# leaner-forever/SEGS-SLAM

Measured on AMD Instinct MI355X. Metric: mapper train-iters/sec (fwd+bwd raster), higher is better.
Workload: dtype f32; 1 GPU; 1080p_3m: 3000000 Gaussians, 1920x1080, 1 keyframe per GPU, fwd+bwd raster; P=3000000, P_visible=2096178, num_rendered=10472370, instances_binned=7913347, instances_live=6766534, width=1920, height=1080, parallelism=keyframe-dp1, forward=resident (no host sync), hipgraph=off

## Files before the change

include/segs_raster.h:

```cpp
#ifndef SEGS_RASTER_H_
#define SEGS_RASTER_H_

#include <stddef.h>
#include <stdint.h>

#ifdef __cplusplus
extern "C" {
#endif

#define SEGS_OK 0
#define SEGS_ERR_INVALID_ARGUMENT (-1)
#define SEGS_ERR_UNSUPPORTED (-2)
#define SEGS_ERR_ALLOC (-3)

typedef char* (*segs_alloc_fn)(void* ctx, size_t bytes);

const char* segs_last_error(void);

#define SEGS_RASTER_SKIP_NONPOSITIVE_OPACITY 1u
#define SEGS_RASTER_KEEP_DEAD_INSTANCES 2u
#define SEGS_RASTER_GATHER_TILES_TOUCHED 4u
#define SEGS_RASTER_TEST_NARROW_PACK 8u
#define SEGS_RASTER_UNFUSED_BINNING 16u
#define SEGS_RASTER_TIGHT_BINNING 32u
#define SEGS_RASTER_MFMA_MOMENTS 64u
#define SEGS_RASTER_NO_WRITTEN_BYTES 128u
#define SEGS_RASTER_UNPACKED_BACKWARD 256u
uint32_t segs_raster_set_flags(uint32_t flags);

uint32_t* segs_raster_set_status_mirror(uint32_t* host_mapped_status);

size_t segs_geometry_bytes(int P);
size_t segs_image_bytes(int width, int height);
size_t segs_binning_bytes(int num_rendered);

int segs_rasterize_forward(segs_alloc_fn geometry_alloc, void* geometry_ctx,
                           segs_alloc_fn binning_alloc, void* binning_ctx,
                           segs_alloc_fn image_alloc, void* image_ctx,
                           int P, int D, int M,
                           const float* background, int width, int height,
                           const float* means3D, const float* shs, const float* colors_precomp,
                           const float* opacities, const float* scales, float scale_modifier,
                           const float* rotations, const float* cov3D_precomp,
                           const float* viewmatrix, const float* projmatrix, const float* cam_pos,
                           float tan_fovx, float tan_fovy, int prefiltered,
                           float* out_color, int* radii, void* stream, int* num_rendered);

int segs_rasterize_backward(int P, int D, int M, int R,
                            const float* background, int width, int height,
                            const float* means3D, const float* shs, const float* colors_precomp,
                            const float* scales, float scale_modifier, const float* rotations,
                            const float* cov3D_precomp, const float* viewmatrix, const float* projmatrix,
                            const float* campos, float tan_fovx, float tan_fovy, const int* radii,
                            char* geom_buffer, char* binning_buffer, char* image_buffer,
                            const float* dL_dpix, float* dL_dmean2D, float* dL_dconic, float* dL_dopacity,
                            float* dL_dcolor, float* dL_dmean3D, float* dL_dcov3D, float* dL_dsh,
                            float* dL_dscale, float* dL_drot, void* stream);

int segs_visible_filter(int P, int M, int width, int height, const float* means3D, const float* scales,
                        float scale_modifier, const float* rotations, const float* cov3D_precomp,
                        const float* viewmatrix, const float* projmatrix, float tan_fovx, float tan_fovy,
                        int prefiltered, int* radii, void* stream);

int segs_visible_filter_log_scales(int P, int width, int height, const float* means3D, const float* scaling_log, int stride,
                                   const float* rotations, const float* viewmatrix, const float* projmatrix, float tan_fovx,
                                   float tan_fovy, int* radii, void* stream);

int segs_mark_visible(int P, const float* means3D, const float* viewmatrix, const float* projmatrix,
                      uint8_t* present, void* stream);

int segs_project2_image(int P, int D, int M, int width, int height, const float* means3D, const float* shs,
                        const float* colors_precomp, const float* opacities, const float* scales,
                        float scale_modifier, const float* rotations, const float* cov3D_precomp,
                        const float* viewmatrix, const float* projmatrix, const float* cam_pos,
                        float tan_fovx, float tan_fovy, int prefiltered, float* out_color, float* points_image,
                        int* radii, void* stream);

int segs_debug_unpack_geometry(const char* geom_buffer, int P, const int* radii, float* means2D ,
                               float* conic_opacity , float* depths , uint32_t* tiles_touched ,
                               uint32_t* point_offsets , float* rgb , void* stream);
int segs_debug_unpack_binning(const char* binning_buffer, const char* geom_buffer, int P, int R, int width, int height,
                              uint64_t* keys_sorted , uint32_t* point_list , void* stream);
int segs_debug_instance_values(const char* binning_buffer, int R, uint32_t* values , void* stream);
int segs_debug_unpack_image(const char* image_buffer, int width, int height, uint32_t* ranges ,
                            float* final_T , uint32_t* n_contrib , void* stream);

#define SEGS_GEOMETRY_REGIONS 10
int segs_debug_geometry_layout(int P, size_t* offset_and_bytes , int regions);

int segs_debug_preprocess_backward(int P, int width, int height, const float* means3D, const int* radii,
                                   const float* scales, float scale_modifier, const float* rotations,
                                   const float* cov3D_precomp, const float* viewmatrix, const float* projmatrix,
                                   float tan_fovx, float tan_fovy, const float* dL_dmean2D, const float* dL_dconic,
                                   float* dL_dmean3D, float* dL_dcov3D, float* dL_dscale, float* dL_drot, void* stream);

int segs_sort_pairs(const uint64_t* keys_in, const uint32_t* vals_in, uint64_t* keys_out, uint32_t* vals_out,
                    int n, int end_bit, char* temp, void* stream);

size_t segs_resident_binning_bytes(int P, int capacity);
int segs_rasterize_forward_resident(char* geom_buffer, char* binning_buffer, char* image_buffer, int capacity,
                                    int geom_rows, int P, int D, int M, const float* background, int width, int height,
                                    const float* means3D, const float* shs, const float* colors_precomp,
                                    const float* opacities, const float* scales, float scale_modifier,
                                    const float* rotations, const float* cov3D_precomp, const float* viewmatrix,
                                    const float* projmatrix, const float* cam_pos, float tan_fovx, float tan_fovy,
                                    float* out_color, int* radii, uint32_t* status, void* stream);
int segs_rasterize_backward_resident(char* geom_buffer, char* binning_buffer, char* image_buffer, int capacity,
                                     int geom_rows, int P, int D, int M, const float* background, int width, int height,
                                     const float* means3D, const float* shs, const float* scales, float scale_modifier,
                                     const float* rotations, const float* cov3D_precomp, const float* viewmatrix,
                                     const float* projmatrix, const float* campos, float tan_fovx, float tan_fovy,
                                     const int* radii, const float* dL_dpix, float* dL_dmean2D, float* dL_dconic,
                                     float* dL_dopacity, float* dL_dcolor, float* dL_dmean3D, float* dL_dcov3D,
                                     float* dL_dsh, float* dL_dscale, float* dL_drot, void* stream);

typedef struct segs_projection_targets {
  float* records;
  int* radii;
  uint32_t* tiles_touched;
  uint32_t* depth_keys;
  uint32_t* tile_ranges;
  uint32_t* depth_overflow;
  int num_tiles;
  uint32_t flags;
} segs_projection_targets;
int segs_resident_projection_targets(char* geom_buffer, char* binning_buffer, char* image_buffer, int capacity, int geom_rows,
                                     int P, int width, int height, int* radii, uint32_t* status, segs_projection_targets* out);
int segs_rasterize_forward_resident_projected(char* geom_buffer, char* binning_buffer, char* image_buffer, int capacity,
                                              int geom_rows, int P, const float* background, int width, int height,
                                              float* out_color, uint32_t* status, void* stream);

typedef struct segs_depth_outputs {
  float* depth;
  float* alpha;
} segs_depth_outputs;
typedef struct segs_depth_grads {
  const float* dL_ddepth;
  const float* dL_dalpha;
} segs_depth_grads;
int segs_rasterize_forward_depth(segs_alloc_fn geometry_alloc, void* geometry_ctx,
                                 segs_alloc_fn binning_alloc, void* binning_ctx,
                                 segs_alloc_fn image_alloc, void* image_ctx,
                                 int P, int D, int M,
                                 const float* background, int width, int height,
                                 const float* means3D, const float* shs, const float* colors_precomp,
                                 const float* opacities, const float* scales, float scale_modifier,
                                 const float* rotations, const float* cov3D_precomp,
                                 const float* viewmatrix, const float* projmatrix, const float* cam_pos,
                                 float tan_fovx, float tan_fovy, int prefiltered,
                                 float* out_color, int* radii, const segs_depth_outputs* depth_out, void* stream,
                                 int* num_rendered);
int segs_rasterize_backward_depth(int P, int D, int M, int R,
                                  const float* background, int width, int height,
                                  const float* means3D, const float* shs, const float* colors_precomp,
                                  const float* scales, float scale_modifier, const float* rotations,
                                  const float* cov3D_precomp, const float* viewmatrix, const float* projmatrix,
                                  const float* campos, float tan_fovx, float tan_fovy, const int* radii,
                                  char* geom_buffer, char* binning_buffer, char* image_buffer,
                                  const float* dL_dpix, float* dL_dmean2D, float* dL_dconic, float* dL_dopacity,
                                  float* dL_dcolor, float* dL_dmean3D, float* dL_dcov3D, float* dL_dsh,
                                  float* dL_dscale, float* dL_drot, const segs_depth_grads* depth_grads, void* stream);
int segs_rasterize_forward_resident_depth(char* geom_buffer, char* binning_buffer, char* image_buffer, int capacity,
                                          int geom_rows, int P, int D, int M, const float* background, int width, int height,
                                          const float* means3D, const float* shs, const float* colors_precomp,
                                          const float* opacities, const float* scales, float scale_modifier,
                                          const float* rotations, const float* cov3D_precomp, const float* viewmatrix,
                                          const float* projmatrix, const float* cam_pos, float tan_fovx, float tan_fovy,
                                          float* out_color, int* radii, uint32_t* status, const segs_depth_outputs* depth_out,
                                          void* stream);
int segs_rasterize_forward_resident_projected_depth(char* geom_buffer, char* binning_buffer, char* image_buffer, int capacity,
                                                    int geom_rows, int P, const float* background, int width, int height,
                                                    float* out_color, uint32_t* status, const segs_depth_outputs* depth_out,
                                                    void* stream);
int segs_rasterize_backward_resident_depth(char* geom_buffer, char* binning_buffer, char* image_buffer, int capacity,
                                           int geom_rows, int P, int D, int M, const float* background, int width, int height,
                                           const float* means3D, const float* shs, const float* scales, float scale_modifier,
                                           const float* rotations, const float* cov3D_precomp, const float* viewmatrix,
                                           const float* projmatrix, const float* campos, float tan_fovx, float tan_fovy,
                                           const int* radii, const float* dL_dpix, float* dL_dmean2D, float* dL_dconic,
                                           float* dL_dopacity, float* dL_dcolor, float* dL_dmean3D, float* dL_dcov3D,
                                           float* dL_dsh, float* dL_dscale, float* dL_drot, const segs_depth_grads* depth_grads,
                                           void* stream);

typedef struct segs_camera_grads {
  float* dL_dviewmatrix;
  float* dL_dprojmatrix;
  char* temp;
} segs_camera_grads;
size_t segs_camera_grad_temp_bytes(int rows);
int segs_rasterize_backward_camera(int P, int D, int M, int R,
                                   const float* background, int width, int height,
                                   const float* means3D, const float* shs, const float* colors_precomp,
                                   const float* scales, float scale_modifier, const float* rotations,
                                   const float* cov3D_precomp, const float* viewmatrix, const float* projmatrix,
                                   const float* campos, float tan_fovx, float tan_fovy, const int* radii,
                                   char* geom_buffer, char* binning_buffer, char* image_buffer,
                                   const float* dL_dpix, float* dL_dmean2D, float* dL_dconic, float* dL_dopacity,
                                   float* dL_dcolor, float* dL_dmean3D, float* dL_dcov3D, float* dL_dsh,
                                   float* dL_dscale, float* dL_drot, const segs_depth_grads* depth_grads,
                                   const segs_camera_grads* camera_grads, void* stream);
int segs_rasterize_backward_resident_camera(char* geom_buffer, char* binning_buffer, char* image_buffer, int capacity,
                                            int geom_rows, int P, int D, int M, const float* background, int width, int height,
                                            const float* means3D, const float* shs, const float* scales, float scale_modifier,
                                            const float* rotations, const float* cov3D_precomp, const float* viewmatrix,
                                            const float* projmatrix, const float* campos, float tan_fovx, float tan_fovy,
                                            const int* radii, const float* dL_dpix, float* dL_dmean2D, float* dL_dconic,
                                            float* dL_dopacity, float* dL_dcolor, float* dL_dmean3D, float* dL_dcov3D,
                                            float* dL_dsh, float* dL_dscale, float* dL_drot, const segs_depth_grads* depth_grads,
                                            const segs_camera_grads* camera_grads, void* stream);
int segs_debug_preprocess_backward_camera(int P, int width, int height, const float* means3D, const int* radii,
                                          const float* scales, float scale_modifier, const float* rotations,
                                          const float* cov3D_precomp, const float* viewmatrix, const float* projmatrix,
                                          float tan_fovx, float tan_fovy, const float* dL_dmean2D, const float* dL_dconic,
                                          float* dL_dmean3D, float* dL_dcov3D, float* dL_dscale, float* dL_drot,
                                          const float* dL_dz, const segs_camera_grads* camera_grads, void* stream);

int segs_profile_begin(unsigned kernel_mask);
int segs_profile_end(void);
int segs_profile_kernel_count(void);
const char* segs_profile_kernel_name(int id);
int segs_profile_query(int id, double* total_ms, long* launches);

#ifdef __cplusplus
}
#endif
#endif
```

segs-slam_amd/_capi.py:

```python
from __future__ import annotations

import ctypes as C
import os
import subprocess

_HERE = os.path.dirname(os.path.abspath(__file__))
CSRC = os.path.join(_HERE, "csrc")
LIB_PATH = os.environ.get("SEGS_RASTER_LIB") or os.path.join(CSRC, "libsegs_raster.so")

ALLOC_FN = C.CFUNCTYPE(C.c_void_p, C.c_void_p, C.c_size_t)


class NeuralDims(C.Structure):
    _fields_ = [("feat_dim", C.c_int), ("n_offsets", C.c_int), ("appearance_dim", C.c_int), ("use_feat_bank", C.c_int),
                ("add_opacity_dist", C.c_int), ("add_cov_dist", C.c_int), ("add_color_dist", C.c_int)]


class ProjectionTargets(C.Structure):
    _fields_ = [("records", C.c_void_p), ("radii", C.c_void_p), ("tiles_touched", C.c_void_p), ("depth_keys", C.c_void_p),
                ("tile_ranges", C.c_void_p), ("depth_overflow", C.c_void_p), ("num_tiles", C.c_int), ("flags", C.c_uint32)]


class DepthOutputs(C.Structure):
    _fields_ = [("depth", C.c_void_p), ("alpha", C.c_void_p)]


class DepthGrads(C.Structure):
    _fields_ = [("dL_ddepth", C.c_void_p), ("dL_dalpha", C.c_void_p)]


class CameraGrads(C.Structure):
    _fields_ = [("dL_dviewmatrix", C.c_void_p), ("dL_dprojmatrix", C.c_void_p), ("temp", C.c_void_p)]


class DepthLossParamsC(C.Structure):
    _fields_ = [("lambda_depth", C.c_float), ("lambda_alpha", C.c_float), ("alpha_min", C.c_float), ("normalize", C.c_int)]


class DepthSeedParamsC(C.Structure):
    _fields_ = [("stride", C.c_int), ("alpha_max", C.c_float), ("use_front", C.c_int), ("front_abs", C.c_float),
                ("front_rel", C.c_float), ("voxel_size", C.c_float)]


class StereoParamsC(C.Structure):
    _fields_ = [("num_disparities", C.c_int), ("min_disparity", C.c_int), ("P1", C.c_int), ("P2", C.c_int),
                ("uniqueness_ratio", C.c_int), ("paths", C.c_int), ("lr_max_diff", C.c_int), ("median", C.c_int)]


class IntakeCameraC(C.Structure):
    _fields_ = [("in_w", C.c_int), ("in_h", C.c_int), ("out_w", C.c_int), ("out_h", C.c_int),
                ("fx", C.c_float), ("fy", C.c_float), ("cx", C.c_float), ("cy", C.c_float),
                ("k1", C.c_float), ("k2", C.c_float), ("p1", C.c_float), ("p2", C.c_float), ("k3", C.c_float),
                ("rinv", C.c_float * 9), ("nfx", C.c_float), ("nfy", C.c_float), ("ncx", C.c_float), ("ncy", C.c_float)]


class AdamSegment(C.Structure):
    _fields_ = [("offset", C.c_int64), ("count", C.c_int64), ("lr", C.c_double)]

_vp, _i, _f, _sz = C.c_void_p, C.c_int, C.c_float, C.c_size_t
SYMBOLS = {
    "segs_last_error": (C.c_char_p, []),
    "segs_raster_set_flags": (C.c_uint, [C.c_uint]),
    "segs_raster_set_status_mirror": (_vp, [_vp]),
    "segs_training_statis": (_i, [_i, _i] + [_vp] * 9),
    "segs_training_statis_guarded": (_i, [_i, _i] + [_vp] * 10),
    "segs_anchor_growing_temp_bytes": (_sz, [_i, _i]),
    "segs_anchor_growing_level": (_i, [_i, _i, _i, _i] + [_vp] * 7 + [_f, _f, _f, _i] + [_vp] * 5),
    "segs_depth_seed_temp_bytes": (_sz, [_i, _i, _i, _i]),
    "segs_depth_seed": (_i, [_i, _vp, _i, _i, _vp, _vp, _vp, _f, _f, _vp, _vp, _i, _vp, _vp, _vp, _vp, _vp]),
    "segs_neural_set_flags": (C.c_uint, [C.c_uint]),
    "segs_neural_param_layout": (_i, [_vp, _vp, _vp, _vp, _vp]),
    "segs_neural_temp_bytes": (_sz, [_vp, _i]),
    "segs_neural_forward": (_i, [_vp, _i] + [_vp] * 16),
    "segs_neural_forward_projected": (_i, [_vp, _i] + [_vp] * 16 + [_i, _i, _f, _f, _f, _vp, _vp]),
    "segs_neural_backward": (_i, [_vp, _i] + [_vp] * 17 + [_f, _vp, _vp, _vp]),
    "segs_neural_backward_camera": (_i, [_vp, _i] + [_vp] * 17 + [_f, _vp, _vp, _vp, _vp]),
    "segs_geometry_bytes": (_sz, [_i]),
    "segs_debug_geometry_layout": (_i, [_i, _vp, _i]),
    "segs_image_bytes": (_sz, [_i, _i]),
    "segs_binning_bytes": (_sz, [_i]),
    "segs_rasterize_forward": (_i, [ALLOC_FN, _vp, ALLOC_FN, _vp, ALLOC_FN, _vp, _i, _i, _i, _vp, _i, _i, _vp, _vp, _vp,
                                     _vp, _vp, _f, _vp, _vp, _vp, _vp, _vp, _f, _f, _i, _vp, _vp, _vp, C.POINTER(_i)]),
    "segs_rasterize_backward": (_i, [_i, _i, _i, _i, _vp, _i, _i, _vp, _vp, _vp, _vp, _f, _vp, _vp, _vp, _vp, _vp, _f, _f,
                                      _vp, _vp, _vp, _vp, _vp, _vp, _vp, _vp, _vp, _vp, _vp, _vp, _vp, _vp, _vp]),
    "segs_resident_binning_bytes": (_sz, [_i, _i]),
    "segs_rasterize_forward_resident": (_i, [_vp, _vp, _vp, _i, _i, _i, _i, _i, _vp, _i, _i, _vp, _vp, _vp, _vp, _vp, _f, _vp, _vp, _vp,
                                              _vp, _vp, _f, _f, _vp, _vp, _vp, _vp]),
    "segs_resident_projection_targets": (_i, [_vp, _vp, _vp, _i, _i, _i, _i, _i, _vp, _vp, _vp]),
    "segs_rasterize_forward_resident_projected": (_i, [_vp, _vp, _vp, _i, _i, _i, _vp, _i, _i, _vp, _vp, _vp]),
    "segs_rasterize_backward_resident": (_i, [_vp, _vp, _vp, _i, _i, _i, _i, _i, _vp, _i, _i, _vp, _vp, _vp, _f, _vp, _vp, _vp, _vp, _vp,
                                               _f, _f, _vp, _vp, _vp, _vp, _vp, _vp, _vp, _vp, _vp, _vp, _vp, _vp]),
}
for _name in ("segs_rasterize_forward", "segs_rasterize_backward", "segs_rasterize_forward_resident",
              "segs_rasterize_forward_resident_projected", "segs_rasterize_backward_resident"):
    _res, _args = SYMBOLS[_name]
    _at = len(_args) - (2 if _name == "segs_rasterize_forward" else 1)
    SYMBOLS[_name + "_depth"] = (_res, _args[:_at] + [_vp] + _args[_at:])
for _name in ("segs_rasterize_backward", "segs_rasterize_backward_resident"):
    _res, _args = SYMBOLS[_name + "_depth"]
    SYMBOLS[_name + "_camera"] = (_res, _args[:-1] + [_vp] + _args[-1:])
SYMBOLS["segs_camera_grad_temp_bytes"] = (_sz, [_i])
SYMBOLS.update({
    "segs_visible_filter": (_i, [_i, _i, _i, _i, _vp, _vp, _f, _vp, _vp, _vp, _vp, _f, _f, _i, _vp, _vp]),
    "segs_visible_filter_log_scales": (_i, [_i, _i, _i, _vp, _vp, _i, _vp, _vp, _vp, _f, _f, _vp, _vp]),
    "segs_mark_visible": (_i, [_i, _vp, _vp, _vp, _vp, _vp]),
    "segs_project2_image": (_i, [_i, _i, _i, _i, _i, _vp, _vp, _vp, _vp, _vp, _f, _vp, _vp, _vp, _vp, _vp, _f, _f, _i,
                                  _vp, _vp, _vp, _vp]),
    "segs_debug_unpack_geometry": (_i, [_vp, _i, _vp, _vp, _vp, _vp, _vp, _vp, _vp, _vp]),
    "segs_debug_instance_values": (_i, [_vp, _i, _vp, _vp]),
    "segs_debug_unpack_binning": (_i, [_vp, _vp, _i, _i, _i, _i, _vp, _vp, _vp]),
    "segs_debug_unpack_image": (_i, [_vp, _i, _i, _vp, _vp, _vp, _vp]),
    "segs_debug_preprocess_backward": (_i, [_i, _i, _i, _vp, _vp, _vp, _f, _vp, _vp, _vp, _vp, _f, _f, _vp, _vp, _vp,
                                             _vp, _vp, _vp, _vp]),
    "segs_debug_preprocess_backward_camera": (_i, [_i, _i, _i, _vp, _vp, _vp, _f, _vp, _vp, _vp, _vp, _f, _f, _vp, _vp, _vp,
                                                    _vp, _vp, _vp, _vp, _vp, _vp]),
    "segs_sort_pairs": (_i, [_vp, _vp, _vp, _vp, _i, _i, _vp, _vp]),
    "segs_knn_temp_bytes": (_sz, [_i]),
    "segs_knn_mean_dist2": (_i, [_i, _vp, _vp, _vp, _vp]),
    "segs_transform_points": (_i, [_i, _vp, _vp, _vp, _vp]),
    "segs_scale_and_transform_points": (_i, [_i, _f, _vp, _vp, _vp, _vp, _vp, _vp, _vp]),
    "segs_reproject_depths_pinhole": (_i, [_i, _i, _f, _f, _f, _f, _vp, _vp, _vp, _vp]),
    "segs_search_neighborhood_depth": (_i, [_i, _i, _f, _f, _f, _f, _f, _vp, _vp, _vp, _vp, _vp, _vp, _vp]),
    "segs_stereo_sgm_temp_bytes": (_sz, [_i, _i, _i, _i]),
    "segs_stereo_sgm": (_i, [_vp, _i, _i, _vp, _vp, _vp, _vp, _f, _vp, _vp]),
    "segs_rgb_to_gray_u8": (_i, [_i, _i, _vp, _vp, _vp]),
    "segs_debug_stereo_sgm_stages": (_i, [_vp, _i, _i, _vp, _vp, _vp, _vp, _f, _vp] + [_vp] * 6 + [_vp]),
    "segs_undistort_u8": (_i, [_vp, _i, _vp, _vp, _vp, _vp]),
    "segs_undistort_depth": (_i, [_vp, _i, _vp, _f, _i, _vp, _vp]),
    "segs_undistort_mask": (_i, [_vp, _vp, _vp]),
    "segs_debug_undistort_map": (_i, [_vp, _vp, _vp]),
    "segs_resize_levels": (_i, [_i, _i, _i, _vp, _i, _vp, _vp, _vp, _vp]),
    "segs_l1_ssim_temp_bytes": (_sz, [_i, _i]),
    "segs_l1_ssim_tile_rows": (_i, [_i, _i]),
    "segs_l1_ssim_loss": (_i, [_vp, _vp, _i, _i, _f, _vp, _vp, _vp, _vp]),
    "segs_freq_pyramid": (_i, [_vp, _i, _i, _i, _i, _vp, _vp, _vp, _vp]),
    "segs_spectrum_magnitude": (_i, [_vp, _sz, _vp, _vp]),
    "segs_freq_temp_bytes": (_sz, [_i, _i, _vp, _vp]),
    "segs_freq_spectrum_loss": (_i, [_i, _i, _vp, _vp, _vp, _vp, _vp, _vp, _vp, _vp, _vp]),
    "segs_freq_pyramid_backward_add": (_i, [_vp, _i, _i, _i, _i, _vp, _vp, _vp, _vp]),
    "segs_freq_plan_create": (_i, [_i, _i, _i, _vp, _f, _vp]),
    "segs_freq_plan_destroy": (None, [_vp]),
    "segs_freq_plan_levels": (_i, [_vp, _vp, _vp, _vp]),
    "segs_freq_target_floats": (_sz, [_vp]),
    "segs_freq_target": (_i, [_vp, _vp, _vp, _vp]),
    "segs_freq_loss": (_i, [_vp, _vp, _vp, _vp, _vp, _vp, _vp]),
    "segs_depth_target_floats": (_sz, [_i, _i]),
    "segs_depth_target": (_i, [_vp, _i, _i, _f, _f, _vp, _vp]),
    "segs_depth_loss_temp_bytes": (_sz, [_i, _i]),
    "segs_depth_loss": (_i, [_vp, _vp, _vp, _i, _i, _vp, _vp, _vp, _vp, _vp, _vp, _vp]),
    "segs_adam_step": (_i, [_vp, _vp, _vp, _vp, _vp, _i, C.c_double, C.c_double, C.c_double, C.c_int64, _f, _i, _vp]),
    "segs_adam_step_guarded": (_i, [_vp, _vp, _vp, _vp, _vp, _i, C.c_double, C.c_double, C.c_double, C.c_int64, _f, _i, _vp, _vp]),
    "segs_adam_step_device": (_i, [_vp, _vp, _vp, _vp, _vp, _i, C.c_double, C.c_double, C.c_double, _vp, _i, _f, _i, _vp, _vp]),
    "segs_adam_step_graph": (_i, [_vp, _vp, _vp, _vp, _vp, _i, _vp, C.c_double, C.c_double, C.c_double, _vp, _f, _i, _vp, _vp]),
    "segs_set_doubles": (_i, [_vp, _vp, _i, _vp]),
    "segs_profile_begin": (_i, [C.c_uint]),
    "segs_profile_end": (_i, []),
    "segs_profile_kernel_count": (_i, []),
    "segs_profile_kernel_name": (C.c_char_p, [_i]),
    "segs_profile_query": (_i, [_i, C.POINTER(C.c_double), C.POINTER(C.c_long)]),
})

_lib = None


def build(force: bool = False) -> str:
    cmd = ["make", "-C", CSRC, "-s", "-j4"] + (["-B"] if force else [])
    subprocess.check_call(cmd)
    return LIB_PATH


def lib() -> C.CDLL:
    global _lib
    if _lib is None:
        if not os.path.exists(LIB_PATH):
            raise RuntimeError(
                f"{LIB_PATH} is missing: the HIP extension must be built (python -c 'import __graft_entry__ as g; "
                "g.build()' or make -C segs-slam_amd/csrc). There is no CPU fallback.")
        import torch
        l = C.CDLL(LIB_PATH)
        for name, (res, args) in SYMBOLS.items():
            try:
                fn = getattr(l, name)
            except AttributeError as e:
                raise RuntimeError(f"libsegs_raster.so does not export {name}") from e
            fn.restype = res
            fn.argtypes = args
        _lib = l
    return _lib


class raster_flags:

    def __init__(self, flags: int, status_mirror=None, clear_mirror: bool = True):
        self.flags, self.status_mirror, self.clear_mirror = flags, status_mirror, clear_mirror

    def __enter__(self):
        self.old = lib().segs_raster_set_flags(self.flags)
        if self.status_mirror is not None:
            _lib.segs_raster_set_status_mirror(self.status_mirror)

    def __exit__(self, *exc):
        _lib.segs_raster_set_flags(self.old)
        if self.clear_mirror:
            _lib.segs_raster_set_status_mirror(None)


class SegsError(RuntimeError):
    pass


def check(status: int, what: str) -> None:
    if status != 0:
        msg = lib().segs_last_error()
        raise SegsError(f"{what} failed with status {status}: {msg.decode() if msg else ''}")
```

segs-slam_amd/csrc/capi.hip:

```cpp
#include <hip/hip_runtime.h>
#include <cstdio>
#include <cstdlib>
#include <algorithm>
#include <cstring>
#include <string>
#include <vector>
#include "../../include/segs_raster.h"
#include "gs_layout.h"
#include "kernels.h"
#include "capi_args.h"

using namespace segs;

namespace {
thread_local std::string g_err;
}
int segs::set_error(int code, const char* what) {
  g_err = what;
  return code;
}
int segs::set_hip_error(hipError_t e, const char* where) {
  g_err = std::string(where) + ": " + hipGetErrorString(e);
  return (int)e > 0 ? (int)e : 1;
}

namespace {

thread_local uint32_t g_flags = 0u;
thread_local uint32_t* g_status_mirror = nullptr;

int fail(int code, const char* what) { return segs::set_error(code, what); }
int hip_fail(hipError_t e, const char* where) { return segs::set_hip_error(e, where); }
#define HIP_TRY(expr)                                   \
  do {                                                  \
    hipError_t _e = (expr);                             \
    if (_e != hipSuccess) return hip_fail(_e, #expr);   \
  } while (0)
#define LAUNCH_TRY(name)                                \
  do {                                                  \
    hipError_t _e = hipGetLastError();                  \
    if (_e != hipSuccess) return hip_fail(_e, name);    \
  } while (0)

enum KernelId { K_PREPROCESS_FWD = 0, K_SCAN, K_DUPLICATE, K_RADIX_COUNT, K_RADIX_SCAN, K_RADIX_SCATTER, K_RANGES,
                K_RENDER_FWD, K_RENDER_BWD, K_PREPROCESS_BWD, K_MEMSET, K_COUNT };
const char* const kKernelNames[K_COUNT] = {"preprocess_fwd_kernel", "scan_block_sums_kernel", "duplicate_with_keys_kernel",
                                           "radix_count_kernel", "radix_scan_kernel", "radix_scatter_kernel",
                                           "identify_tile_ranges_kernel", "render_fwd_kernel", "render_bwd_kernel",
                                           "preprocess_bwd_kernel", "memset"};
struct Profiler {
  unsigned mask = 0;
  std::vector<hipEvent_t> pool;
  size_t used = 0;
  struct Span { int id; size_t e0, e1; };
  std::vector<Span> spans;
  double total_ms[K_COUNT] = {0};
  long count[K_COUNT] = {0};
  hipEvent_t get() {
    if (used == pool.size()) { hipEvent_t e; if (hipEventCreate(&e) != hipSuccess) return nullptr; pool.push_back(e); }
    return pool[used++];
  }
} g_prof;
struct ProfScope {
  int id; hipStream_t st; size_t e0 = 0; bool on;
  ProfScope(int id_, hipStream_t st_) : id(id_), st(st_), on((g_prof.mask >> id_) & 1u) {
    if (on) { e0 = g_prof.used; hipEvent_t e = g_prof.get(); if (e) (void)hipEventRecord(e, st); else on = false; }
  }
  ~ProfScope() {
    if (on) { size_t e1 = g_prof.used; hipEvent_t e = g_prof.get(); if (e) { (void)hipEventRecord(e, st); g_prof.spans.push_back({id, e0, e1}); } }
  }
};
#define PROF(id) ProfScope _prof_scope_##id(id, st)

uint32_t getHigherMsb(uint32_t n) {
  uint32_t msb = sizeof(n) * 4, step = msb;
  while (step > 1) {
    step /= 2;
    if (n >> msb) msb += step; else msb -= step;
  }
  if (n >> msb) msb++;
  return msb;
}

int count_chunk_tiles(int nblocks) {
#ifdef SEGS_MEASURE
  static const int chunk_override = [] { const char* e = getenv("SEGS_COUNT_CHUNK"); const int v = e ? atoi(e) : 0; return (v == 1 || v == 2 || v == 4) ? v : 0; }();
  if (chunk_override > 0) return chunk_override;
#endif
  return nblocks <= 256 ? 1 : (nblocks <= 2048 ? 2 : SORT_COUNT_CHUNK_TILES);
}

int check_tile_grid(const View& V) {
  if (V.gx > 0xFFFFu || V.gy > 0xFFFFu) return fail(SEGS_ERR_INVALID_ARGUMENT, "image too large for 16-bit tile coordinates");
  return SEGS_OK;
}
int check_colour_and_shape(const Gaussians& g, const View& V) {
  if (!g.colors_precomp && (!g.shs || !V.cam_pos || g.M <= 0 || g.D < 0 || (g.D + 1) * (g.D + 1) > g.M || g.D > 3))
    return fail(SEGS_ERR_INVALID_ARGUMENT, "need colors_precomp, or shs + cam_pos with (D+1)^2 <= M, D <= 3");
  if (!g.cov3D_precomp && (!g.scales || !g.rotations)) return fail(SEGS_ERR_INVALID_ARGUMENT, "need scales+rotations or cov3D_precomp");
  return SEGS_OK;
}

template <typename K, int BITS>
int sort_pairs_digits(char* bin, const BinningLayout& L, int n, const SortOptions& o, hipStream_t st) {
  if (n <= 0) return SEGS_OK;
  uint32_t* n_live = (uint32_t*)(bin + L.n_live);
  const int end_bit = o.end_bit, passes = (end_bit + BITS - 1) / BITS;
  int side = sort_first_side(end_bit, BITS);
  uint32_t* tile_prefix = (uint32_t*)(bin + L.tile_prefix);
  uint32_t* chunk_hist = (uint32_t*)(bin + L.chunk_hist);
  uint32_t* digit_totals = (uint32_t*)(bin + L.digit_totals);
  const int chunk_tiles = count_chunk_tiles(L.nblocks);
  const int nchunks = (L.nblocks + chunk_tiles - 1) / chunk_tiles;
  for (int p = 0; p < passes; p++) {
    const K* kin = (p == 0 && o.first_keys) ? (const K*)o.first_keys : (const K*)(bin + L.keys[side]);
    const uint32_t* vin = (const uint32_t*)(bin + L.vals[side]);
    K* kout = (K*)(bin + L.keys[side ^ 1]);
    uint32_t* vout = (uint32_t*)(bin + L.vals[side ^ 1]);
    const int shift = BITS * p;
    const int drop = o.drop_dead && p == 0;
    const uint32_t* n_in = (o.drop_dead && p > 0) ? n_live : o.n_dev;
    const int nbits = std::min(BITS, end_bit - shift);
    { PROF(K_RADIX_COUNT);
    radix_count_kernel<K, BITS><<<(nchunks + 7) / 8 * 8, SORT_THREADS, 0, st>>>(kin, n, shift, o.dmin, o.dbits, tile_prefix, chunk_hist, L.nblocks, nchunks, n_in, drop, chunk_tiles, nbits);
    }
    LAUNCH_TRY("radix_count_kernel");
    const bool last = p == passes - 1;
    { PROF(K_RADIX_SCAN);
    radix_scan_kernel<<<1 << BITS, 256, 0, st>>>(chunk_hist, nchunks, digit_totals);
    }
    LAUNCH_TRY("radix_scan_kernel");
    if (o.iota_vals && p == 0) vin = nullptr;
    const int scatter_grid = (L.nblocks + 7) / 8 * 8;
    uint2* fr = last ? o.ranges : nullptr;
    uint32_t* fs = last ? o.status : nullptr;
    uint32_t* fm = last ? o.status_mirror : nullptr;
    const int wk = (last && !o.keep_sorted_keys) ? 0 : 1;
    { PROF(K_RADIX_SCATTER);
    bool gathered = false;
    if constexpr (sizeof(K) == 4 && BITS <= 9) {
      if (o.aux_in && o.aux_final && last) {
        radix_scatter_kernel<K, BITS, true><<<scatter_grid, SORT_THREADS, 0, st>>>(kin, vin, kout, vout, n, shift, o.dmin, o.dbits, tile_prefix, chunk_hist,
                                                                        digit_totals, L.nblocks, nchunks, n_in, drop,
                                                                        drop ? n_live : nullptr, o.aux_in, o.aux_final, nbits, chunk_tiles, 0, fr, fs, fm, wk);
        gathered = true;
      }
    }
    if (!gathered)
      radix_scatter_kernel<K, BITS, false><<<scatter_grid, SORT_THREADS, 0, st>>>(kin, vin, kout, vout, n, shift, o.dmin, o.dbits, tile_prefix, chunk_hist,
                                                                       digit_totals, L.nblocks, nchunks, n_in, drop,
                                                                       drop ? n_live : nullptr, (o.pack_shift > 0 && p == 0) ? o.aux_in : nullptr, nullptr,
                                                                       nbits, chunk_tiles, (p == 0) ? o.pack_shift : 0, fr, fs, fm, wk);
    }
    LAUNCH_TRY("radix_scatter_kernel");
    side ^= 1;
  }
  return SEGS_OK;
}
template <typename K>
int sort_pairs(char* bin, const BinningLayout& L, int n, const SortOptions& o, hipStream_t st) {
  if constexpr (sizeof(K) == 4) {
    if (o.digit_bits == 9) return sort_pairs_digits<K, 9>(bin, L, n, o, st);
    if (o.digit_bits == 11) return sort_pairs_digits<K, 11>(bin, L, n, o, st);
  }
  return sort_pairs_digits<K, 8>(bin, L, n, o, st);
}

bool drop_dead_instances() { return (g_flags & SEGS_RASTER_KEEP_DEAD_INSTANCES) == 0u; }
uint32_t resident_k1_flags() { return drop_dead_instances() ? PREPROCESS_TIGHT_RECT : 0u; }

int run_preprocess(const Geom& G, const Gaussians& g, const View& V, int* radii, const K1Targets& k1, hipStream_t st) {
  { PROF(K_PREPROCESS_FWD);
  preprocess_fwd_kernel<<<G.L.nblocks, 256, 0, st>>>(g.P, g.means3D, g.kernel_scales(), g.scale_modifier, g.rotations, g.opacities, g.colors_precomp,
                                                     g.cov3D_precomp, V.viewmatrix, V.projmatrix, V.width, V.height, V.tan_fovx, V.tan_fovy,
                                                     V.focal_x, V.focal_y, V.gx, V.gy, radii, G.rec(), G.bin(), G.block_sums(),
                                                     G.block_sums() + (G.L.nblocks + 1), g.shs, g.D, g.M, V.cam_pos, G.clamped(),
                                                     g_flags | k1.extra_flags, k1.depth_keys, k1.depth_vals, k1.ranges, (int)V.tiles,
                                                     k1.depth_overflow, G.touched());
  }
  LAUNCH_TRY("preprocess_fwd_kernel");
  return SEGS_OK;
}

int run_binning(const Scratch& S, const View& V, const BinningMode& mode, hipStream_t st) {
  const Geom& G = S.G; const BinningLayout& BL = S.BL; const GaussSortLayout& GS = S.GS;
  char* const bin = S.bin; uint2* const ranges = S.ranges();
  const int P = G.L.P, n_cap = BL.R;
  const uint32_t* const n_dev = S.status;
  uint32_t* const total_out = S.status ? S.status : (uint32_t*)(bin + GS.block_sums) + G.L.nblocks;
  const int bit = (int)getHigherMsb(V.tiles);
  char* gbin = bin + GS.base;
  const BinningLayout& GL = GS.inner;
  if (!mode.k1_keys) { PROF(K_DUPLICATE);
  const DepthSortInput in = depth_sort_input(bin, GS, mode.dbits, mode.digit_bits);
  make_depth_keys_kernel<<<G.L.nblocks, 256, 0, st>>>(P, G.bin(), mode.dcull, in.keys, in.vals, ranges, (int)V.tiles);
  }
  LAUNCH_TRY("make_depth_keys_kernel");
  const bool drop_culled = mode.k1_keys != nullptr;
  int idx_bits = 1;
  while (idx_bits < 32 && ((uint64_t)1 << idx_bits) < (uint64_t)P) idx_bits++;
  int pack_shift = (32 - idx_bits >= 6 && !(g_flags & SEGS_RASTER_GATHER_TILES_TOUCHED)) ? idx_bits : 0;
  if (pack_shift && (g_flags & SEGS_RASTER_TEST_NARROW_PACK)) pack_shift = 30;
  SortOptions depth_sort;
  depth_sort.end_bit = mode.dbits; depth_sort.digit_bits = mode.digit_bits;
  depth_sort.dmin = mode.dmin; depth_sort.dbits = mode.dbits;
  depth_sort.drop_dead = drop_culled; depth_sort.iota_vals = true;
  depth_sort.aux_in = G.touched(); depth_sort.aux_final = pack_shift ? nullptr : G.offsets(); depth_sort.pack_shift = pack_shift;
  depth_sort.first_keys = mode.k1_keys;
  int rc = sort_pairs<uint32_t>(gbin, GL, P, depth_sort, st);
  if (rc) return rc;
  uint32_t* order = (uint32_t*)(gbin + GL.vals[0]);
  const uint32_t* ng_dev = drop_culled ? (const uint32_t*)(gbin + GL.n_live) : nullptr;
  uint32_t* sums2 = (uint32_t*)(bin + GS.block_sums);
  uint32_t* first_owner = (uint32_t*)(bin + GS.first_owner);
  const int prefix_wgs = (P + 256 * PREFIX_ROWS_PER_WG - 1) / (256 * PREFIX_ROWS_PER_WG);
  { PROF(K_SCAN);
  ordered_block_sums_kernel<<<prefix_wgs, 256, 0, st>>>(P, pack_shift ? G.touched() : G.offsets(), nullptr, sums2, G.offsets(), ng_dev, order, pack_shift);
  }
  LAUNCH_TRY("ordered_block_sums_kernel");
#ifdef SEGS_MEASURE
  static const bool no_wide = getenv("SEGS_NO_WIDE_DIGIT") != nullptr;
#else
  constexpr bool no_wide = false;
#endif
  SortOptions tile_sort;
  tile_sort.end_bit = bit;
  tile_sort.digit_bits = (!no_wide && bit <= 11 && BL.nblocks <= SORT_WIDE_MAX_TILES) ? 11 : 8;
  tile_sort.n_dev = n_dev; tile_sort.drop_dead = mode.drop_dead;
  const int tpasses = (bit + tile_sort.digit_bits - 1) / tile_sort.digit_bits;
  const int side = sort_first_side(bit, tile_sort.digit_bits);
  { PROF(K_SCAN);
  ordered_offsets_kernel<<<prefix_wgs, 256, 0, st>>>(P, sums2, G.offsets(), total_out, ng_dev, first_owner,
                                                      (uint32_t)(n_cap / EMIT_SLOTS_PER_WG + 2));
  }
  LAUNCH_TRY("ordered_offsets_kernel");
  const bool unfused = (g_flags & SEGS_RASTER_UNFUSED_BINNING) != 0u;
  { PROF(K_DUPLICATE);
  duplicate_with_keys_kernel<<<(n_cap + EMIT_SLOTS_PER_WG - 1) / EMIT_SLOTS_PER_WG, 256, 0, st>>>(P, n_cap, G.rec(), order, G.offsets(),
                                                                    (uint32_t*)(bin + BL.keys[side]), (uint32_t*)(bin + BL.vals[side]), V.gx, n_dev,
                                                                    mode.drop_dead ? 1 : 0, ng_dev, first_owner);
  }
  LAUNCH_TRY("duplicate_with_keys_kernel");
  const bool fused_ranges = !unfused && tpasses >= 2;
  if (fused_ranges) {
    tile_sort.ranges = ranges;
    tile_sort.status = n_dev ? total_out : nullptr;
    tile_sort.status_mirror = n_dev ? g_status_mirror : nullptr;
    tile_sort.keep_sorted_keys = n_dev == nullptr;
  }
  rc = sort_pairs<uint32_t>(bin, BL, n_cap, tile_sort, st);
  if (rc) return rc;
  if (!fused_ranges) { PROF(K_RANGES);
  identify_tile_ranges_kernel<<<(n_cap + 256 * RANGE_KEYS_PER_THREAD - 1) / (256 * RANGE_KEYS_PER_THREAD), 256, 0, st>>>(n_cap, (const uint32_t*)(bin + BL.keys[0]), ranges, n_dev,
                                                                   n_dev ? total_out : nullptr, n_dev ? g_status_mirror : nullptr,
                                                                   mode.drop_dead ? (const uint32_t*)(bin + BL.n_live) : nullptr);
  }
  LAUNCH_TRY("identify_tile_ranges_kernel");
  return SEGS_OK;
}

int launch_render_fwd(const Scratch& S, const View& V, const float* background, float* out_color, const segs_depth_outputs* dout,
                      hipStream_t st) {
  PROF(K_RENDER_FWD);
  if (dout && (dout->depth || dout->alpha))
    render_fwd_depth_kernel<<<V.tiles, 256, 0, st>>>(S.ranges(), S.point_list(), V.width, V.height, S.G.rec(), background, S.final_T(),
                                                     S.n_contrib(), out_color, dout->depth, dout->alpha);
  else
    render_fwd_kernel<<<V.tiles, 256, 0, st>>>(S.ranges(), S.point_list(), V.width, V.height, S.G.rec(), background, S.final_T(), S.n_contrib(),
                                               out_color);
  LAUNCH_TRY("render_fwd_kernel");
  return SEGS_OK;
}

int launch_render_bwd(const Scratch& S, const View& V, const float* background, const float* dL_dpix, const segs_depth_grads* dgrad,
                      uint8_t* written, hipStream_t st) {
  PROF(K_RENDER_BWD);
  const uint32_t grid = (V.tiles + 7) / 8 * 32;
  if (dgrad && (dgrad->dL_ddepth || dgrad->dL_dalpha)) {
    render_bwd_depth_kernel<<<grid, 64, 0, st>>>(S.ranges(), S.point_list(), V.width, V.height, S.G.rec(), background, S.final_T(),
                                                 S.n_contrib(), dL_dpix, S.G.gacc(), V.tiles, dgrad->dL_ddepth, dgrad->dL_dalpha, written);
    LAUNCH_TRY("render_bwd_depth_kernel");
    return SEGS_OK;
  }
  static const bool mfma_env = [] { const char* e = getenv("SEGS_RENDER_BWD_MFMA"); return e && e[0] == '1'; }();
  ((mfma_env || (g_flags & SEGS_RASTER_MFMA_MOMENTS)) ? render_bwd_mfma_kernel : render_bwd_kernel)<<<grid, 64, 0, st>>>(
      S.ranges(), S.point_list(), V.width, V.height, S.G.rec(), background, S.final_T(), S.n_contrib(), dL_dpix, S.G.gacc(), V.tiles, written);
  LAUNCH_TRY("render_bwd_kernel");
  return SEGS_OK;
}

int camera_grads_begin(const segs_camera_grads* cam, const float* shs, bool empty, hipStream_t st, bool* live) {
  *live = false;
  if (!cam) return SEGS_OK;
  if (!cam->dL_dviewmatrix || !cam->dL_dprojmatrix || !cam->temp) return fail(SEGS_ERR_INVALID_ARGUMENT, "segs_camera_grads: null field");
  if (shs) return fail(SEGS_ERR_INVALID_ARGUMENT, "camera gradients need colors_precomp: the SH colours depend on campos, which they do not cover");
  if (empty) {
    HIP_TRY(hipMemsetAsync(cam->dL_dviewmatrix, 0, 16 * sizeof(float), st));
    HIP_TRY(hipMemsetAsync(cam->dL_dprojmatrix, 0, 16 * sizeof(float), st));
    return SEGS_OK;
  }
  *live = true;
  return SEGS_OK;
}
float* camera_partials(const segs_camera_grads* cam) { return (float*)align_ptr(cam->temp); }
int camera_grads_finish(const segs_camera_grads* cam, int nblocks, hipStream_t st) {
  camera_grad_reduce_kernel<<<1, 960, 0, st>>>(camera_partials(cam), nblocks, cam->dL_dviewmatrix, cam->dL_dprojmatrix);
  LAUNCH_TRY("camera_grad_reduce_kernel");
  return SEGS_OK;
}

int launch_preprocess_bwd(const Gaussians& g, const View& V, const int* radii, const GradOutputs& o, const PerGaussianBwd& m, hipStream_t st) {
  const bool depth = m.depth || m.dz_in;
  auto* const kernel = m.cam ? (depth ? preprocess_bwd_kernel<true, true> : preprocess_bwd_kernel<false, true>)
                             : (depth ? preprocess_bwd_kernel<true, false> : preprocess_bwd_kernel<false, false>);
  const int nblocks = (g.P + 255) / 256;
  if (m.packed) {
    auto* const packed = m.cam ? (depth ? preprocess_bwd_packed_kernel<true, true> : preprocess_bwd_packed_kernel<false, true>)
                               : (depth ? preprocess_bwd_packed_kernel<true, false> : preprocess_bwd_packed_kernel<false, false>);
    packed<<<nblocks, 256, 0, st>>>(g.P, g.means3D, radii, g.kernel_scales(), g.rotations, g.scale_modifier, g.cov3D_precomp, V.viewmatrix,
                                    V.projmatrix, V.focal_x, V.focal_y, V.tan_fovx, V.tan_fovy, m.gacc, (float)V.width, (float)V.height,
                                    o.dL_dmean2D, o.dL_dconic, o.dL_dopacity, o.dL_dcolor, o.dL_dmean3D, o.dL_dcov3D, o.dL_dscale, o.dL_drot,
                                    m.cam ? camera_partials(m.cam) : nullptr, m.written);
    LAUNCH_TRY("preprocess_bwd_packed_kernel");
    return m.cam ? camera_grads_finish(m.cam, nblocks, st) : SEGS_OK;
  }
  kernel<<<nblocks, 256, 0, st>>>(g.P, g.means3D, radii, g.kernel_scales(), g.rotations, g.scale_modifier, g.cov3D_precomp, V.viewmatrix,
                                  V.projmatrix, V.focal_x, V.focal_y, V.tan_fovx, V.tan_fovy, m.gacc, (float)V.width, (float)V.height,
                                  o.dL_dmean2D, o.dL_dconic, o.dL_dopacity, o.dL_dcolor, o.dL_dmean3D, o.dL_dcov3D, o.dL_dscale, o.dL_drot,
                                  m.clean_gacc ? 1 : 0, m.dz_in, m.cam ? camera_partials(m.cam) : nullptr, m.written);
  LAUNCH_TRY("preprocess_bwd_kernel");
  return m.cam ? camera_grads_finish(m.cam, nblocks, st) : SEGS_OK;
}

int rasterize_forward(const Allocators& A, const Gaussians& g, const View& V, const float* background, float* out_color, int* radii,
                      const segs_depth_outputs* dout, hipStream_t st, int* num_rendered) {
  const int P = g.P;
  if (!A.geometry_alloc || !A.binning_alloc || !A.image_alloc) return fail(SEGS_ERR_INVALID_ARGUMENT, "null allocator callback");
  if (P < 0 || V.width <= 0 || V.height <= 0) return fail(SEGS_ERR_INVALID_ARGUMENT, "bad P / image size");
  if (P > MAX_GAUSSIANS) return fail(SEGS_ERR_INVALID_ARGUMENT, "P exceeds 2^28 Gaussians (sort values carry a 4-bit quadrant mask)");
  if (!background || !out_color || !V.viewmatrix || !V.projmatrix || !num_rendered) return fail(SEGS_ERR_INVALID_ARGUMENT, "null required pointer");
  if (P > 0 && (!g.means3D || !g.opacities)) return fail(SEGS_ERR_INVALID_ARGUMENT, "null means3D/opacities");
  if (P > 0)
    if (int rc = check_colour_and_shape(g, V)) return rc;
  if (int rc = check_tile_grid(V)) return rc;

  Scratch S{};
  char* geom_raw = A.geometry_alloc(A.geometry_ctx, geom_layout(P).total);
  S.IL = image_layout(V.width, V.height);
  char* img_raw = A.image_alloc(A.image_ctx, S.IL.total);
  if (!geom_raw || !img_raw) return fail(SEGS_ERR_ALLOC, "allocator callback returned null");
  S.G = geom_at(geom_raw, P);
  S.img = align_ptr(img_raw);
  const Geom& G = S.G;
  if (!radii) radii = G.radii_internal();

  int R = 0;
  uint32_t hdr[3] = {0u, 0u, 0u};
  const bool tight = (g_flags & SEGS_RASTER_TIGHT_BINNING) != 0u;
  bool fast_keys = tight;
  if (P > 0) {
    K1Targets k1;
    k1.extra_flags = tight ? PREPROCESS_TIGHT_RECT : 0u;
    if (fast_keys) { k1.depth_keys = (uint32_t*)G.bin(); k1.ranges = S.ranges(); }
    int rc = run_preprocess(G, g, V, radii, k1, st);
    if (rc) return rc;
    { PROF(K_SCAN);
    scan_block_sums_kernel<<<1, 1024, 0, st>>>(G.block_sums(), G.L.nblocks, G.block_sums() + (G.L.nblocks + 1), G.num_rendered());
    }
    LAUNCH_TRY("scan_block_sums_kernel");
    HIP_TRY(hipMemcpyAsync(hdr, G.num_rendered(), sizeof(hdr), hipMemcpyDeviceToHost, st));
    HIP_TRY(hipStreamSynchronize(st));
    R = (int)hdr[0];
    if (R < 0) return fail(SEGS_ERR_INVALID_ARGUMENT, "num_rendered overflows int32");
    if (fast_keys && R > 0 && (hdr[2] - DEPTH_KEY_MIN) >= ((1u << DEPTH_KEY_BITS) - 1u)) {
      fast_keys = false;
      K1Targets exact;
      exact.extra_flags = PREPROCESS_TIGHT_RECT;
      rc = run_preprocess(G, g, V, radii, exact, st);
      if (rc) return rc;
    }
  }
  S.BL = binning_layout(R);
  S.GS = gauss_sort_layout(R, P);
  char* bin_raw = A.binning_alloc(A.binning_ctx, S.GS.total);
  if (!bin_raw) return fail(SEGS_ERR_ALLOC, "binning allocator returned null");
  S.bin = align_ptr(bin_raw);

  if (R == 0) {
    PROF(K_MEMSET);
    HIP_TRY(hipMemsetAsync(S.ranges(), 0, (size_t)V.gx * V.gy * sizeof(uint2), st));
  }
  if (R > 0) {
    const BinningMode mode = fast_keys ? BinningMode::resident_keys((const uint32_t*)G.bin(), tight)
                                       : BinningMode::exact_range(hdr[1], hdr[2], tight);
    if (int rc = run_binning(S, V, mode, st)) return rc;
  }
  if (int rc = launch_render_fwd(S, V, background, out_color, dout, st)) return rc;
  *num_rendered = R;
  return SEGS_OK;
}

int open_resident(const ScratchBuffers& B, int P, const View& V, uint32_t* status, bool others_present, const Gaussians* k1, Scratch* S) {
  if (P <= 0 || B.capacity <= 0 || V.width <= 0 || V.height <= 0) return fail(SEGS_ERR_INVALID_ARGUMENT, "bad sizes");
  if (B.geom_rows < P) return fail(SEGS_ERR_INVALID_ARGUMENT, "geom_rows (rows the geometry buffer was sized for) must be >= P");
  if (B.geom_rows > MAX_GAUSSIANS) return fail(SEGS_ERR_INVALID_ARGUMENT, "P exceeds 2^28 Gaussians");
  if (!B.geom_buffer || !B.binning_buffer || !B.image_buffer || !status || !others_present) return fail(SEGS_ERR_INVALID_ARGUMENT, "null required pointer");
  if (k1)
    if (int rc = check_colour_and_shape(*k1, V)) return rc;
  if (int rc = check_tile_grid(V)) return rc;
  *S = carve(B, P, V, status);
  return SEGS_OK;
}

int rasterize_forward_resident(const ScratchBuffers& B, int P, const Gaussians* k1, const View& V, const float* background, float* out_color,
                               int* radii, uint32_t* status, const segs_depth_outputs* dout, hipStream_t st) {
  Scratch S{};
  const bool others_present = background && out_color && (!k1 || (V.viewmatrix && V.projmatrix && k1->means3D && k1->opacities));
  if (int rc = open_resident(B, P, V, status, others_present, k1, &S)) return rc;
  const DepthSortInput keys = resident_depth_sort_input(S.bin, S.GS);
  if (k1) {
    K1Targets t;
    t.depth_keys = keys.keys; t.depth_vals = keys.vals; t.ranges = S.ranges();
    t.extra_flags = resident_k1_flags(); t.depth_overflow = status + 2;
    if (int rc = run_preprocess(S.G, *k1, V, radii ? radii : S.G.radii_internal(), t, st)) return rc;
  }
  if (int rc = run_binning(S, V, BinningMode::resident_keys(keys.keys, drop_dead_instances()), st)) return rc;
  return launch_render_fwd(S, V, background, out_color, dout, st);
}

int rasterize_backward(const Gaussians& g, const View& V, const ScratchBuffers& B, const BackwardInputs& in, const GradOutputs& o,
                       GaccCleaning cleaning, hipStream_t st) {
  const int P = g.P, R = B.capacity;
  const bool self_clean = cleaning == SELF_CLEAN;
  if (P < 0 || R < 0 || V.width <= 0 || V.height <= 0) return fail(SEGS_ERR_INVALID_ARGUMENT, "bad sizes");
  if (B.geom_rows < P) return fail(SEGS_ERR_INVALID_ARGUMENT, "geom_rows must be >= P");
  bool cam_live = false;
  if (int rc = camera_grads_begin(in.cam, g.shs, P == 0 || R == 0, st, &cam_live)) return rc;
  if (P == 0) return SEGS_OK;
  if (g.shs && (!V.cam_pos || !o.dL_dsh || g.M <= 0)) return fail(SEGS_ERR_INVALID_ARGUMENT, "SH path needs campos, dL_dsh and M > 0");
  if (!B.geom_buffer || !B.binning_buffer || !B.image_buffer || !in.dL_dpix || !in.background || !g.means3D || !V.viewmatrix || !V.projmatrix)
    return fail(SEGS_ERR_INVALID_ARGUMENT, "null required pointer");
  if (!o.dL_dmean2D || !o.dL_dopacity || !o.dL_dcolor || !o.dL_dmean3D || (g.cov3D_precomp && !o.dL_dcov3D))
    return fail(SEGS_ERR_INVALID_ARGUMENT, "null gradient output");
  if (!g.cov3D_precomp && (!g.scales || !g.rotations || !o.dL_dscale || !o.dL_drot))
    return fail(SEGS_ERR_INVALID_ARGUMENT, "need scales+rotations (+ their gradient outputs) or cov3D_precomp");
  uint32_t* const no_status = nullptr;
  const Scratch S = carve(B, P, V, no_status);
  const Geom& G = S.G;
  const int* radii = in.radii ? in.radii : G.radii_internal();

  if (!self_clean) { PROF(K_MEMSET);
  HIP_TRY(hipMemsetAsync(G.gacc(), 0, (size_t)P * GACC_DWORDS * 4, st));
  }
  PerGaussianBwd m;
  m.gacc = G.gacc(); m.depth = in.dgrad && in.dgrad->dL_ddepth; m.clean_gacc = self_clean;
  if (cam_live) m.cam = in.cam;
  m.written = (self_clean && !(g_flags & SEGS_RASTER_NO_WRITTEN_BYTES)) ? G.written() : nullptr;
  m.packed = m.written && !(g_flags & SEGS_RASTER_UNPACKED_BACKWARD);
  if (R > 0)
    if (int rc = launch_render_bwd(S, V, in.background, in.dL_dpix, in.dgrad, m.written, st)) return rc;
  { PROF(K_PREPROCESS_BWD);
  if (int rc = launch_preprocess_bwd(g, V, radii, o, m, st)) return rc;
  }
  if (g.shs) {
    sh_backward_kernel<<<G.L.nblocks, 256, 0, st>>>(P, g.means3D, radii, g.shs, g.D, g.M, V.cam_pos, G.clamped(), o.dL_dcolor, o.dL_dmean3D, o.dL_dsh);
    LAUNCH_TRY("sh_backward_kernel");
  }
  return SEGS_OK;
}

int visible_filter(const Gaussians& g, const View& V, int log_scale_stride, int* radii, hipStream_t st) {
  if (g.P < 0 || V.width <= 0 || V.height <= 0) return fail(SEGS_ERR_INVALID_ARGUMENT, "bad sizes");
  if (g.P == 0) return SEGS_OK;
  if (!g.means3D || !V.viewmatrix || !V.projmatrix || !radii) return fail(SEGS_ERR_INVALID_ARGUMENT, "null required pointer");
  if (!g.cov3D_precomp && (!g.scales || !g.rotations)) return fail(SEGS_ERR_INVALID_ARGUMENT, "need scales+rotations or cov3D_precomp");
  visible_filter_kernel<<<(g.P + 255) / 256, 256, 0, st>>>(g.P, g.means3D, g.kernel_scales(), g.scale_modifier, g.rotations, g.cov3D_precomp,
                                                           V.viewmatrix, V.projmatrix, V.width, V.height, V.tan_fovx, V.tan_fovy, V.focal_x,
                                                           V.focal_y, V.gx, V.gy, radii, log_scale_stride);
  LAUNCH_TRY("visible_filter_kernel");
  return SEGS_OK;
}

int debug_preprocess_backward(const Gaussians& g, const View& V, const int* radii, const GradOutputs& o, const float* dL_dz,
                              const segs_camera_grads* cam, hipStream_t st) {
  bool cam_live = false;
  if (int rc = camera_grads_begin(cam, g.shs, g.P <= 0, st, &cam_live)) return rc;
  if (g.P <= 0) return SEGS_OK;
  if (!g.means3D || !radii || !V.viewmatrix || !V.projmatrix || !o.dL_dmean2D || !o.dL_dconic || !o.dL_dmean3D || !o.dL_dcov3D)
    return fail(SEGS_ERR_INVALID_ARGUMENT, "null pointer");
  PerGaussianBwd m;
  if (cam_live) { m.dz_in = dL_dz; m.cam = cam; }
  return launch_preprocess_bwd(g, V, radii, o, m, st);
}

}

extern "C" {

const char* segs_last_error(void) { return g_err.c_str(); }

uint32_t* segs_raster_set_status_mirror(uint32_t* host_mapped_status) {
  uint32_t* old = g_status_mirror;
  g_status_mirror = host_mapped_status;
  return old;
}

uint32_t segs_raster_set_flags(uint32_t flags) {
  const uint32_t old = g_flags;
  g_flags = flags;
  return old;
}

size_t segs_geometry_bytes(int P) { return geom_layout(P < 0 ? 0 : P).total; }
size_t segs_image_bytes(int width, int height) { return image_layout(width, height).total; }

int segs_debug_geometry_layout(int P, size_t* offset_and_bytes, int regions) {
  if (P < 0 || !offset_and_bytes || regions != SEGS_GEOMETRY_REGIONS) return fail(SEGS_ERR_INVALID_ARGUMENT, "bad P / region count");
  const GeomLayout g = geom_layout(P);
  const size_t p = (size_t)P;
  const size_t v[SEGS_GEOMETRY_REGIONS][2] = {
      {g.rec, p * REC_DWORDS * 4}, {g.bin, p * sizeof(BinInfo)}, {g.offsets, p * 4}, {g.radii_internal, p * 4},
      {g.block_sums, (size_t)(g.nblocks + 1) * 4 * 3}, {g.clamped, p * 4}, {g.num_rendered, 64}, {g.gacc, p * GACC_DWORDS * 4},
      {g.touched, p * 4}, {g.written, p}};
  for (int i = 0; i < SEGS_GEOMETRY_REGIONS; i++) { offset_and_bytes[2 * i] = v[i][0]; offset_and_bytes[2 * i + 1] = v[i][1]; }
  return SEGS_OK;
}
size_t segs_binning_bytes(int num_rendered) { return binning_layout(num_rendered < 0 ? 0 : num_rendered).total; }

int segs_rasterize_forward(segs_alloc_fn geometry_alloc, void* geometry_ctx, segs_alloc_fn binning_alloc, void* binning_ctx,
                           segs_alloc_fn image_alloc, void* image_ctx, int P, int D, int M, const float* background,
                           int width, int height, const float* means3D, const float* shs, const float* colors_precomp,
                           const float* opacities, const float* scales, float scale_modifier, const float* rotations,
                           const float* cov3D_precomp, const float* viewmatrix, const float* projmatrix,
                           const float* cam_pos, float tan_fovx, float tan_fovy, int prefiltered, float* out_color,
                           int* radii, void* stream, int* num_rendered) {
  (void)prefiltered;
  return rasterize_forward(Allocators{geometry_alloc, geometry_ctx, binning_alloc, binning_ctx, image_alloc, image_ctx},
                           Gaussians{P, means3D, scales, scale_modifier, rotations, cov3D_precomp, D, M, shs, colors_precomp, opacities},
                           camera_view(width, height, viewmatrix, projmatrix, cam_pos, tan_fovx, tan_fovy), background, out_color, radii,
                           NO_DEPTH_OUTPUTS, (hipStream_t)stream, num_rendered);
}

int segs_rasterize_forward_depth(segs_alloc_fn geometry_alloc, void* geometry_ctx, segs_alloc_fn binning_alloc, void* binning_ctx,
                                 segs_alloc_fn image_alloc, void* image_ctx, int P, int D, int M, const float* background,
                                 int width, int height, const float* means3D, const float* shs, const float* colors_precomp,
                                 const float* opacities, const float* scales, float scale_modifier, const float* rotations,
                                 const float* cov3D_precomp, const float* viewmatrix, const float* projmatrix,
                                 const float* cam_pos, float tan_fovx, float tan_fovy, int prefiltered, float* out_color,
                                 int* radii, const segs_depth_outputs* depth_out, void* stream, int* num_rendered) {
  (void)prefiltered;
  return rasterize_forward(Allocators{geometry_alloc, geometry_ctx, binning_alloc, binning_ctx, image_alloc, image_ctx},
                           Gaussians{P, means3D, scales, scale_modifier, rotations, cov3D_precomp, D, M, shs, colors_precomp, opacities},
                           camera_view(width, height, viewmatrix, projmatrix, cam_pos, tan_fovx, tan_fovy), background, out_color, radii,
                           depth_out, (hipStream_t)stream, num_rendered);
}

int segs_rasterize_backward(int P, int D, int M, int R, const float* background, int width, int height,
                            const float* means3D, const float* shs, const float* colors_precomp, const float* scales,
                            float scale_modifier, const float* rotations, const float* cov3D_precomp,
                            const float* viewmatrix, const float* projmatrix, const float* campos, float tan_fovx,
                            float tan_fovy, const int* radii, char* geom_buffer, char* binning_buffer, char* image_buffer,
                            const float* dL_dpix, float* dL_dmean2D, float* dL_dconic, float* dL_dopacity, float* dL_dcolor,
                            float* dL_dmean3D, float* dL_dcov3D, float* dL_dsh, float* dL_dscale, float* dL_drot, void* stream) {
  (void)colors_precomp;
  return rasterize_backward(Gaussians{P, means3D, scales, scale_modifier, rotations, cov3D_precomp, D, M, shs},
                            camera_view(width, height, viewmatrix, projmatrix, campos, tan_fovx, tan_fovy),
                            ScratchBuffers{geom_buffer, binning_buffer, image_buffer, R, P},
                            BackwardInputs{background, radii, dL_dpix, NO_DEPTH_GRADS, NO_CAMERA_GRADS},
                            GradOutputs{dL_dmean2D, dL_dconic, dL_dmean3D, dL_dcov3D, dL_dscale, dL_drot, dL_dopacity, dL_dcolor, dL_dsh},
                            MEMSET_PER_CALL, (hipStream_t)stream);
}

int segs_rasterize_backward_depth(int P, int D, int M, int R, const float* background, int width, int height,
                                  const float* means3D, const float* shs, const float* colors_precomp, const float* scales,
                                  float scale_modifier, const float* rotations, const float* cov3D_precomp,
                                  const float* viewmatrix, const float* projmatrix, const float* campos, float tan_fovx,
                                  float tan_fovy, const int* radii, char* geom_buffer, char* binning_buffer, char* image_buffer,
                                  const float* dL_dpix, float* dL_dmean2D, float* dL_dconic, float* dL_dopacity, float* dL_dcolor,
                                  float* dL_dmean3D, float* dL_dcov3D, float* dL_dsh, float* dL_dscale, float* dL_drot,
                                  const segs_depth_grads* depth_grads, void* stream) {
  (void)colors_precomp;
  return rasterize_backward(Gaussians{P, means3D, scales, scale_modifier, rotations, cov3D_precomp, D, M, shs},
                            camera_view(width, height, viewmatrix, projmatrix, campos, tan_fovx, tan_fovy),
                            ScratchBuffers{geom_buffer, binning_buffer, image_buffer, R, P},
                            BackwardInputs{background, radii, dL_dpix, depth_grads, NO_CAMERA_GRADS},
                            GradOutputs{dL_dmean2D, dL_dconic, dL_dmean3D, dL_dcov3D, dL_dscale, dL_drot, dL_dopacity, dL_dcolor, dL_dsh},
                            MEMSET_PER_CALL, (hipStream_t)stream);
}

size_t segs_camera_grad_temp_bytes(int rows) { return align_up((size_t)((rows < 0 ? 0 : rows) + 255) / 256 * CAM_SUMS * sizeof(float)) + ALIGN; }

int segs_rasterize_backward_camera(int P, int D, int M, int R, const float* background, int width, int height,
                                   const float* means3D, const float* shs, const float* colors_precomp, const float* scales,
                                   float scale_modifier, const float* rotations, const float* cov3D_precomp,
                                   const float* viewmatrix, const float* projmatrix, const float* campos, float tan_fovx,
                                   float tan_fovy, const int* radii, char* geom_buffer, char* binning_buffer, char* image_buffer,
                                   const float* dL_dpix, float* dL_dmean2D, float* dL_dconic, float* dL_dopacity, float* dL_dcolor,
                                   float* dL_dmean3D, float* dL_dcov3D, float* dL_dsh, float* dL_dscale, float* dL_drot,
                                   const segs_depth_grads* depth_grads, const segs_camera_grads* camera_grads, void* stream) {
  (void)colors_precomp;
  return rasterize_backward(Gaussians{P, means3D, scales, scale_modifier, rotations, cov3D_precomp, D, M, shs},
                            camera_view(width, height, viewmatrix, projmatrix, campos, tan_fovx, tan_fovy),
                            ScratchBuffers{geom_buffer, binning_buffer, image_buffer, R, P},
                            BackwardInputs{background, radii, dL_dpix, depth_grads, camera_grads},
                            GradOutputs{dL_dmean2D, dL_dconic, dL_dmean3D, dL_dcov3D, dL_dscale, dL_drot, dL_dopacity, dL_dcolor, dL_dsh},
                            MEMSET_PER_CALL, (hipStream_t)stream);
}

int segs_visible_filter(int P, int M, int width, int height, const float* means3D, const float* scales,
                        float scale_modifier, const float* rotations, const float* cov3D_precomp, const float* viewmatrix,
                        const float* projmatrix, float tan_fovx, float tan_fovy, int prefiltered, int* radii, void* stream) {
  (void)M; (void)prefiltered;
  return visible_filter(Gaussians{P, means3D, scales, scale_modifier, rotations, cov3D_precomp},
                        camera_view(width, height, viewmatrix, projmatrix, NO_CAM_POS, tan_fovx, tan_fovy), 0, radii, (hipStream_t)stream);
}

int segs_visible_filter_log_scales(int P, int width, int height, const float* means3D, const float* scaling_log, int stride,
                                   const float* rotations, const float* viewmatrix, const float* projmatrix, float tan_fovx,
                                   float tan_fovy, int* radii, void* stream) {
  if (stride < 3 || !scaling_log || !rotations) return fail(SEGS_ERR_INVALID_ARGUMENT, "need log-scales (stride >= 3) and rotations");
  return visible_filter(Gaussians{P, means3D, scaling_log, 1.0f, rotations},
                        camera_view(width, height, viewmatrix, projmatrix, NO_CAM_POS, tan_fovx, tan_fovy), stride, radii, (hipStream_t)stream);
}

int segs_mark_visible(int P, const float* means3D, const float* viewmatrix, const float* projmatrix, uint8_t* present, void* stream) {
  (void)projmatrix;
  hipStream_t st = (hipStream_t)stream;
  if (P < 0) return fail(SEGS_ERR_INVALID_ARGUMENT, "bad P");
  if (P == 0) return SEGS_OK;
  if (!means3D || !viewmatrix || !present) return fail(SEGS_ERR_INVALID_ARGUMENT, "null required pointer");
  mark_visible_kernel<<<(P + 255) / 256, 256, 0, st>>>(P, means3D, viewmatrix, present);
  LAUNCH_TRY("mark_visible_kernel");
  return SEGS_OK;
}

int segs_debug_unpack_geometry(const char* geom_buffer, int P, const int* radii, float* means2D, float* conic_opacity,
                               float* depths, uint32_t* tiles_touched, uint32_t* point_offsets, float* rgb, void* stream) {
  hipStream_t st = (hipStream_t)stream;
  if (P <= 0) return SEGS_OK;
  if (!geom_buffer || !means2D || !conic_opacity || !depths || !tiles_touched) return fail(SEGS_ERR_INVALID_ARGUMENT, "null pointer");
  Geom G = geom_at(const_cast<char*>(geom_buffer), P);
  if (!radii) radii = G.radii_internal();
  unpack_geometry_kernel<<<(P + 255) / 256, 256, 0, st>>>(P, G.rec(), G.bin(), radii, means2D, conic_opacity, depths, tiles_touched, rgb);
  LAUNCH_TRY("unpack_geometry_kernel");
  if (point_offsets) {
    point_offsets_kernel<<<1, 1024, 0, st>>>(P, G.bin(), point_offsets);
    LAUNCH_TRY("point_offsets_kernel");
  }
  return SEGS_OK;
}

int segs_debug_unpack_binning(const char* binning_buffer, const char* geom_buffer, int P, int R, int width, int height,
                              uint64_t* keys_sorted, uint32_t* point_list, void* stream) {
  (void)width; (void)height;
  hipStream_t st = (hipStream_t)stream;
  if (R <= 0) return SEGS_OK;
  if (!binning_buffer || (keys_sorted && (!geom_buffer || P <= 0))) return fail(SEGS_ERR_INVALID_ARGUMENT, "null pointer");
  const BinningLayout BL = binning_layout(R);
  const char* bin = align_ptr(binning_buffer);
  if (keys_sorted) {
    const Geom G = geom_at(const_cast<char*>(geom_buffer), P);
    rebuild_keys_kernel<<<(R + 255) / 256, 256, 0, st>>>(R, (const uint32_t*)(bin + BL.keys[0]), (const uint32_t*)(bin + BL.vals[0]),
                                                        G.bin(), keys_sorted);
    LAUNCH_TRY("rebuild_keys_kernel");
  }
  if (point_list) {
    strip_mask_kernel<<<(R + 255) / 256, 256, 0, st>>>(R, (const uint32_t*)(bin + BL.vals[0]), point_list);
    LAUNCH_TRY("strip_mask_kernel");
  }
  return SEGS_OK;
}

int segs_debug_instance_values(const char* binning_buffer, int R, uint32_t* values, void* stream) {
  if (R <= 0) return SEGS_OK;
  if (!binning_buffer || !values) return fail(SEGS_ERR_INVALID_ARGUMENT, "null pointer");
  const BinningLayout BL = binning_layout(R);
  HIP_TRY(hipMemcpyAsync(values, align_ptr(binning_buffer) + BL.vals[0], (size_t)R * 4, hipMemcpyDeviceToDevice, (hipStream_t)stream));
  return SEGS_OK;
}

int segs_debug_unpack_image(const char* image_buffer, int width, int height, uint32_t* ranges, float* final_T,
                            uint32_t* n_contrib, void* stream) {
  hipStream_t st = (hipStream_t)stream;
  if (!image_buffer) return fail(SEGS_ERR_INVALID_ARGUMENT, "null pointer");
  const ImageLayout IL = image_layout(width, height);
  const char* img = align_ptr(image_buffer);
  const size_t tiles = image_view(width, height).tiles;
  if (ranges) {
    HIP_TRY(hipMemcpyAsync(ranges, img + IL.ranges, tiles * 8, hipMemcpyDeviceToDevice, st));
    normalize_ranges_kernel<<<(int)((tiles + 255) / 256), 256, 0, st>>>((int)tiles, (uint2*)ranges);
    LAUNCH_TRY("normalize_ranges_kernel");
  }
  if (final_T) HIP_TRY(hipMemcpyAsync(final_T, img + IL.final_T, (size_t)width * height * 4, hipMemcpyDeviceToDevice, st));
  if (n_contrib) HIP_TRY(hipMemcpyAsync(n_contrib, img + IL.n_contrib, (size_t)width * height * 4, hipMemcpyDeviceToDevice, st));
  return SEGS_OK;
}

int segs_debug_preprocess_backward(int P, int width, int height, const float* means3D, const int* radii, const float* scales,
                                   float scale_modifier, const float* rotations, const float* cov3D_precomp,
                                   const float* viewmatrix, const float* projmatrix, float tan_fovx, float tan_fovy,
                                   const float* dL_dmean2D, const float* dL_dconic, float* dL_dmean3D, float* dL_dcov3D,
                                   float* dL_dscale, float* dL_drot, void* stream) {
  return debug_preprocess_backward(Gaussians{P, means3D, scales, scale_modifier, rotations, cov3D_precomp},
                                   camera_view(width, height, viewmatrix, projmatrix, NO_CAM_POS, tan_fovx, tan_fovy), radii,
                                   GradOutputs{const_cast<float*>(dL_dmean2D), const_cast<float*>(dL_dconic), dL_dmean3D, dL_dcov3D, dL_dscale, dL_drot}, NO_DL_DZ,
                                   NO_CAMERA_GRADS, (hipStream_t)stream);
}

int segs_debug_preprocess_backward_camera(int P, int width, int height, const float* means3D, const int* radii, const float* scales,
                                          float scale_modifier, const float* rotations, const float* cov3D_precomp,
                                          const float* viewmatrix, const float* projmatrix, float tan_fovx, float tan_fovy,
                                          const float* dL_dmean2D, const float* dL_dconic, float* dL_dmean3D, float* dL_dcov3D,
                                          float* dL_dscale, float* dL_drot, const float* dL_dz, const segs_camera_grads* camera_grads,
                                          void* stream) {
  return debug_preprocess_backward(Gaussians{P, means3D, scales, scale_modifier, rotations, cov3D_precomp},
                                   camera_view(width, height, viewmatrix, projmatrix, NO_CAM_POS, tan_fovx, tan_fovy), radii,
                                   GradOutputs{const_cast<float*>(dL_dmean2D), const_cast<float*>(dL_dconic), dL_dmean3D, dL_dcov3D, dL_dscale, dL_drot}, dL_dz, camera_grads,
                                   (hipStream_t)stream);
}

int segs_sort_pairs(const uint64_t* keys_in, const uint32_t* vals_in, uint64_t* keys_out, uint32_t* vals_out, int n,
                    int end_bit, char* temp, void* stream) {
  hipStream_t st = (hipStream_t)stream;
  if (n < 0 || end_bit <= 0 || end_bit > 64) return fail(SEGS_ERR_INVALID_ARGUMENT, "bad n / end_bit");
  if (n == 0) return SEGS_OK;
  if (!keys_in || !vals_in || !keys_out || !vals_out || !temp) return fail(SEGS_ERR_INVALID_ARGUMENT, "null pointer");
  const BinningLayout BL = binning_layout(n);
  char* bin = align_ptr(temp);
  SortOptions sort;
  sort.end_bit = end_bit; sort.dbits = 32;
  const int side = sort_first_side(end_bit, sort.digit_bits);
  HIP_TRY(hipMemcpyAsync(bin + BL.keys[side], keys_in, (size_t)n * 8, hipMemcpyDeviceToDevice, st));
  HIP_TRY(hipMemcpyAsync(bin + BL.vals[side], vals_in, (size_t)n * 4, hipMemcpyDeviceToDevice, st));
  int rc = sort_pairs<uint64_t>(bin, BL, n, sort, st);
  if (rc) return rc;
  HIP_TRY(hipMemcpyAsync(keys_out, bin + BL.keys[0], (size_t)n * 8, hipMemcpyDeviceToDevice, st));
  HIP_TRY(hipMemcpyAsync(vals_out, bin + BL.vals[0], (size_t)n * 4, hipMemcpyDeviceToDevice, st));
  return SEGS_OK;
}

int segs_project2_image(int P, int D, int M, int width, int height, const float* means3D, const float* shs,
                        const float* colors_precomp, const float* opacities, const float* scales, float scale_modifier,
                        const float* rotations, const float* cov3D_precomp, const float* viewmatrix, const float* projmatrix,
                        const float* cam_pos, float tan_fovx, float tan_fovy, int prefiltered, float* out_color,
                        float* points_image, int* radii, void* stream) {
  (void)prefiltered;
  hipStream_t st = (hipStream_t)stream;
  if (P < 0 || width <= 0 || height <= 0) return fail(SEGS_ERR_INVALID_ARGUMENT, "bad sizes");
  if (P == 0) return SEGS_OK;
  if (!colors_precomp && (!shs || !cam_pos || M <= 0)) return fail(SEGS_ERR_INVALID_ARGUMENT, "need colors_precomp or shs + cam_pos");
  if (!means3D || !opacities || !viewmatrix || !projmatrix || !out_color || !points_image || !radii)
    return fail(SEGS_ERR_INVALID_ARGUMENT, "null required pointer");
  const GeomLayout GL = geom_layout(P);
  char* raw = nullptr;
  HIP_TRY(hipMallocAsync((void**)&raw, GL.total + (size_t)P * 4 * 8, st));
  Geom G = geom_at(raw, P);
  float* tmp = (float*)(align_ptr(raw) + GL.total - ALIGN);
  int rc = run_preprocess(G, Gaussians{P, means3D, scales, scale_modifier, rotations, cov3D_precomp, D, M, shs, colors_precomp, opacities},
                          camera_view(width, height, viewmatrix, projmatrix, cam_pos, tan_fovx, tan_fovy), radii, K1Targets(), st);
  if (rc == SEGS_OK) {
    unpack_geometry_kernel<<<(P + 255) / 256, 256, 0, st>>>(P, G.rec(), G.bin(), radii, points_image, tmp, tmp + (size_t)4 * P,
                                                            (uint32_t*)(tmp + (size_t)5 * P), out_color);
    hipError_t e = hipGetLastError();
    if (e != hipSuccess) rc = hip_fail(e, "unpack_geometry_kernel");
  }
  hipError_t fe = hipFreeAsync(raw, st);
  if (rc == SEGS_OK && fe != hipSuccess) return hip_fail(fe, "hipFreeAsync");
  return rc;
}


size_t segs_resident_binning_bytes(int P, int capacity) { return gauss_sort_layout(capacity < 0 ? 0 : capacity, P < 0 ? 0 : P).total; }

int segs_rasterize_forward_resident(char* geom_buffer, char* binning_buffer, char* image_buffer, int capacity, int geom_rows, int P, int D, int M,
                                    const float* background, int width, int height, const float* means3D, const float* shs,
                                    const float* colors_precomp, const float* opacities, const float* scales, float scale_modifier,
                                    const float* rotations, const float* cov3D_precomp, const float* viewmatrix,
                                    const float* projmatrix, const float* cam_pos, float tan_fovx, float tan_fovy, float* out_color,
                                    int* radii, uint32_t* status, void* stream) {
  const Gaussians g{P, means3D, scales, scale_modifier, rotations, cov3D_precomp, D, M, shs, colors_precomp, opacities};
  return rasterize_forward_resident(ScratchBuffers{geom_buffer, binning_buffer, image_buffer, capacity, geom_rows}, P, &g,
                                    camera_view(width, height, viewmatrix, projmatrix, cam_pos, tan_fovx, tan_fovy), background, out_color,
                                    radii, status, NO_DEPTH_OUTPUTS, (hipStream_t)stream);
}

int segs_rasterize_forward_resident_depth(char* geom_buffer, char* binning_buffer, char* image_buffer, int capacity, int geom_rows, int P,
                                          int D, int M, const float* background, int width, int height, const float* means3D,
                                          const float* shs, const float* colors_precomp, const float* opacities, const float* scales,
                                          float scale_modifier, const float* rotations, const float* cov3D_precomp,
                                          const float* viewmatrix, const float* projmatrix, const float* cam_pos, float tan_fovx,
                                          float tan_fovy, float* out_color, int* radii, uint32_t* status,
                                          const segs_depth_outputs* depth_out, void* stream) {
  const Gaussians g{P, means3D, scales, scale_modifier, rotations, cov3D_precomp, D, M, shs, colors_precomp, opacities};
  return rasterize_forward_resident(ScratchBuffers{geom_buffer, binning_buffer, image_buffer, capacity, geom_rows}, P, &g,
                                    camera_view(width, height, viewmatrix, projmatrix, cam_pos, tan_fovx, tan_fovy), background, out_color,
                                    radii, status, depth_out, (hipStream_t)stream);
}

int segs_resident_projection_targets(char* geom_buffer, char* binning_buffer, char* image_buffer, int capacity, int geom_rows, int P,
                                     int width, int height, int* radii, uint32_t* status, segs_projection_targets* out) {
  if (!out) return fail(SEGS_ERR_INVALID_ARGUMENT, "bad sizes");
  const View V = image_view(width, height);
  Scratch S{};
  const bool nothing_else_required = true;
  if (int rc = open_resident(ScratchBuffers{geom_buffer, binning_buffer, image_buffer, capacity, geom_rows}, P, V, status, nothing_else_required,
                             K1_RAN_AT_PRODUCER, &S))
    return rc;
  out->records = S.G.rec();
  out->radii = radii ? radii : S.G.radii_internal();
  out->tiles_touched = S.G.touched();
  out->depth_keys = resident_depth_sort_input(S.bin, S.GS).keys;
  out->tile_ranges = (uint32_t*)S.ranges();
  out->depth_overflow = status + 2;
  out->num_tiles = (int)V.tiles;
  out->flags = resident_k1_flags();
  return SEGS_OK;
}

int segs_rasterize_forward_resident_projected(char* geom_buffer, char* binning_buffer, char* image_buffer, int capacity, int geom_rows, int P,
                                              const float* background, int width, int height, float* out_color, uint32_t* status,
                                              void* stream) {
  return rasterize_forward_resident(ScratchBuffers{geom_buffer, binning_buffer, image_buffer, capacity, geom_rows}, P, K1_RAN_AT_PRODUCER,
                                    image_view(width, height), background, out_color, NO_RADII, status, NO_DEPTH_OUTPUTS, (hipStream_t)stream);
}

int segs_rasterize_forward_resident_projected_depth(char* geom_buffer, char* binning_buffer, char* image_buffer, int capacity,
                                                    int geom_rows, int P, const float* background, int width, int height,
                                                    float* out_color, uint32_t* status, const segs_depth_outputs* depth_out,
                                                    void* stream) {
  return rasterize_forward_resident(ScratchBuffers{geom_buffer, binning_buffer, image_buffer, capacity, geom_rows}, P, K1_RAN_AT_PRODUCER,
                                    image_view(width, height), background, out_color, NO_RADII, status, depth_out, (hipStream_t)stream);
}

int segs_rasterize_backward_resident(char* geom_buffer, char* binning_buffer, char* image_buffer, int capacity, int geom_rows, int P, int D, int M,
                                     const float* background, int width, int height, const float* means3D, const float* shs,
                                     const float* scales, float scale_modifier, const float* rotations, const float* cov3D_precomp,
                                     const float* viewmatrix, const float* projmatrix, const float* campos, float tan_fovx,
                                     float tan_fovy, const int* radii, const float* dL_dpix, float* dL_dmean2D, float* dL_dconic,
                                     float* dL_dopacity, float* dL_dcolor, float* dL_dmean3D, float* dL_dcov3D, float* dL_dsh,
                                     float* dL_dscale, float* dL_drot, void* stream) {
  return rasterize_backward(Gaussians{P, means3D, scales, scale_modifier, rotations, cov3D_precomp, D, M, shs},
                            camera_view(width, height, viewmatrix, projmatrix, campos, tan_fovx, tan_fovy),
                            ScratchBuffers{geom_buffer, binning_buffer, image_buffer, capacity, geom_rows},
                            BackwardInputs{background, radii, dL_dpix, NO_DEPTH_GRADS, NO_CAMERA_GRADS},
                            GradOutputs{dL_dmean2D, dL_dconic, dL_dmean3D, dL_dcov3D, dL_dscale, dL_drot, dL_dopacity, dL_dcolor, dL_dsh},
                            SELF_CLEAN, (hipStream_t)stream);
}

int segs_rasterize_backward_resident_depth(char* geom_buffer, char* binning_buffer, char* image_buffer, int capacity, int geom_rows, int P,
                                           int D, int M, const float* background, int width, int height, const float* means3D,
                                           const float* shs, const float* scales, float scale_modifier, const float* rotations,
                                           const float* cov3D_precomp, const float* viewmatrix, const float* projmatrix,
                                           const float* campos, float tan_fovx, float tan_fovy, const int* radii, const float* dL_dpix,
                                           float* dL_dmean2D, float* dL_dconic, float* dL_dopacity, float* dL_dcolor, float* dL_dmean3D,
                                           float* dL_dcov3D, float* dL_dsh, float* dL_dscale, float* dL_drot,
                                           const segs_depth_grads* depth_grads, void* stream) {
  return rasterize_backward(Gaussians{P, means3D, scales, scale_modifier, rotations, cov3D_precomp, D, M, shs},
                            camera_view(width, height, viewmatrix, projmatrix, campos, tan_fovx, tan_fovy),
                            ScratchBuffers{geom_buffer, binning_buffer, image_buffer, capacity, geom_rows},
                            BackwardInputs{background, radii, dL_dpix, depth_grads, NO_CAMERA_GRADS},
                            GradOutputs{dL_dmean2D, dL_dconic, dL_dmean3D, dL_dcov3D, dL_dscale, dL_drot, dL_dopacity, dL_dcolor, dL_dsh},
                            SELF_CLEAN, (hipStream_t)stream);
}

int segs_rasterize_backward_resident_camera(char* geom_buffer, char* binning_buffer, char* image_buffer, int capacity, int geom_rows, int P,
                                            int D, int M, const float* background, int width, int height, const float* means3D,
                                            const float* shs, const float* scales, float scale_modifier, const float* rotations,
                                            const float* cov3D_precomp, const float* viewmatrix, const float* projmatrix,
                                            const float* campos, float tan_fovx, float tan_fovy, const int* radii, const float* dL_dpix,
                                            float* dL_dmean2D, float* dL_dconic, float* dL_dopacity, float* dL_dcolor, float* dL_dmean3D,
                                            float* dL_dcov3D, float* dL_dsh, float* dL_dscale, float* dL_drot,
                                            const segs_depth_grads* depth_grads, const segs_camera_grads* camera_grads, void* stream) {
  return rasterize_backward(Gaussians{P, means3D, scales, scale_modifier, rotations, cov3D_precomp, D, M, shs},
                            camera_view(width, height, viewmatrix, projmatrix, campos, tan_fovx, tan_fovy),
                            ScratchBuffers{geom_buffer, binning_buffer, image_buffer, capacity, geom_rows},
                            BackwardInputs{background, radii, dL_dpix, depth_grads, camera_grads},
                            GradOutputs{dL_dmean2D, dL_dconic, dL_dmean3D, dL_dcov3D, dL_dscale, dL_drot, dL_dopacity, dL_dcolor, dL_dsh},
                            SELF_CLEAN, (hipStream_t)stream);
}

int segs_profile_begin(unsigned kernel_mask) {
  g_prof.mask = kernel_mask; g_prof.used = 0; g_prof.spans.clear();
  for (int i = 0; i < K_COUNT; i++) { g_prof.total_ms[i] = 0; g_prof.count[i] = 0; }
  return SEGS_OK;
}
int segs_profile_end(void) {
  g_prof.mask = 0;
  for (const auto& sp : g_prof.spans) {
    HIP_TRY(hipEventSynchronize(g_prof.pool[sp.e1]));
    float ms = 0.f;
    HIP_TRY(hipEventElapsedTime(&ms, g_prof.pool[sp.e0], g_prof.pool[sp.e1]));
    g_prof.total_ms[sp.id] += ms; g_prof.count[sp.id]++;
  }
  g_prof.spans.clear(); g_prof.used = 0;
  return SEGS_OK;
}
int segs_profile_kernel_count(void) { return K_COUNT; }
const char* segs_profile_kernel_name(int id) { return (id >= 0 && id < K_COUNT) ? kKernelNames[id] : ""; }
int segs_profile_query(int id, double* total_ms, long* launches) {
  if (id < 0 || id >= K_COUNT || !total_ms || !launches) return fail(SEGS_ERR_INVALID_ARGUMENT, "bad profile query");
  *total_ms = g_prof.total_ms[id]; *launches = g_prof.count[id];
  return SEGS_OK;
}

}
```

segs-slam_amd/csrc/capi_args.h:

```cpp
#pragma once
#include <hip/hip_runtime.h>
#include <cstdint>
#include "../../include/segs_raster.h"
#include "gs_layout.h"
#include "kernels.h"

namespace segs {

struct Gaussians {
  int P; const float *means3D, *scales; float scale_modifier; const float *rotations, *cov3D_precomp;
  int D, M; const float *shs, *colors_precomp, *opacities;
  const float* kernel_scales() const { return cov3D_precomp ? nullptr : scales; }
};

struct View {
  int width, height; const float *viewmatrix, *projmatrix, *cam_pos; float tan_fovx, tan_fovy;
  uint32_t gx, gy, tiles; float focal_x, focal_y;
};
inline View image_view(int width, int height) {
  View v{};
  v.width = width; v.height = height;
  v.gx = (width + TILE_X - 1) / TILE_X; v.gy = (height + TILE_Y - 1) / TILE_Y; v.tiles = v.gx * v.gy;
  return v;
}
inline View camera_view(int width, int height, const float* viewmatrix, const float* projmatrix, const float* cam_pos, float tan_fovx, float tan_fovy) {
  View v = image_view(width, height);
  v.viewmatrix = viewmatrix; v.projmatrix = projmatrix; v.cam_pos = cam_pos; v.tan_fovx = tan_fovx; v.tan_fovy = tan_fovy;
  v.focal_y = height / (2.0f * tan_fovy);
  v.focal_x = width / (2.0f * tan_fovx);
  return v;
}

struct GradOutputs { float *dL_dmean2D, *dL_dconic, *dL_dmean3D, *dL_dcov3D, *dL_dscale, *dL_drot, *dL_dopacity, *dL_dcolor, *dL_dsh; };
struct ScratchBuffers { char *geom_buffer, *binning_buffer, *image_buffer; int capacity, geom_rows; };

inline int sort_first_side(int end_bit, int digit_bits) { return ((end_bit + digit_bits - 1) / digit_bits) & 1; }
struct SortOptions {
  int end_bit = 0;
  int digit_bits = 8;
  uint32_t dmin = 0u; int dbits = 0;
  const uint32_t* n_dev = nullptr;
  bool drop_dead = false;
  bool iota_vals = false;
  const uint32_t* aux_in = nullptr;
  uint32_t* aux_final = nullptr;
  int pack_shift = 0;
  const void* first_keys = nullptr;
  uint2* ranges = nullptr;
  uint32_t* status = nullptr;
  uint32_t* status_mirror = nullptr;
  bool keep_sorted_keys = true;
};

struct Geom {
  GeomLayout L;
  char* base;
  float* rec() const { return (float*)(base + L.rec); }
  BinInfo* bin() const { return (BinInfo*)(base + L.bin); }
  uint32_t* offsets() const { return (uint32_t*)(base + L.offsets); }
  int* radii_internal() const { return (int*)(base + L.radii_internal); }
  uint32_t* block_sums() const { return (uint32_t*)(base + L.block_sums); }
  uint32_t* num_rendered() const { return (uint32_t*)(base + L.num_rendered); }
  uint32_t* clamped() const { return (uint32_t*)(base + L.clamped); }
  float* gacc() const { return (float*)(base + L.gacc); }
  uint32_t* touched() const { return (uint32_t*)(base + L.touched); }
  uint8_t* written() const { return (uint8_t*)(base + L.written); }
};
inline Geom geom_at(char* p, int P) { return Geom{geom_layout(P), align_ptr(p)}; }
inline Geom geom_at(char* p, int P, int rows) {
  Geom g{geom_layout(rows), align_ptr(p)};
  g.L.P = P;
  g.L.nblocks = (P + 255) / 256;
  return g;
}

struct Scratch {
  Geom G;
  char *img, *bin;
  ImageLayout IL;
  BinningLayout BL;
  GaussSortLayout GS;
  uint32_t* status;
  uint2* ranges() const { return (uint2*)(img + IL.ranges); }
  const uint32_t* point_list() const { return (const uint32_t*)(bin + BL.vals[0]); }
  float* final_T() const { return (float*)(img + IL.final_T); }
  uint32_t* n_contrib() const { return (uint32_t*)(img + IL.n_contrib); }
};
inline Scratch carve(const ScratchBuffers& B, int P, const View& V, uint32_t* status) {
  return Scratch{geom_at(B.geom_buffer, P, B.geom_rows), align_ptr(B.image_buffer), align_ptr(B.binning_buffer), image_layout(V.width, V.height),
                 binning_layout(B.capacity), gauss_sort_layout(B.capacity, P), status};
}

struct DepthSortInput { uint32_t *keys, *vals; };
inline DepthSortInput depth_sort_input(char* bin, const GaussSortLayout& GS, int dbits, int digit_bits) {
  const int side = sort_first_side(dbits, digit_bits);
  return DepthSortInput{(uint32_t*)(bin + GS.base + GS.inner.keys[side]), (uint32_t*)(bin + GS.base + GS.inner.vals[side])};
}

struct BinningMode {
  uint32_t dmin; int dbits; uint32_t dcull;
  int digit_bits;
  const uint32_t* k1_keys;
  bool drop_dead;
  static constexpr int RESIDENT_DIGIT_BITS = 9;
  static BinningMode resident_keys(const uint32_t* k1_keys, bool drop_dead) {
    return BinningMode{DEPTH_KEY_MIN, DEPTH_KEY_BITS, 0xFFFFFFFFu, RESIDENT_DIGIT_BITS, k1_keys, drop_dead};
  }
  static BinningMode exact_range(uint32_t max_not_depth, uint32_t max_depth, bool drop_dead) {
    const uint32_t dmin = ~max_not_depth, dspan = max_depth - dmin + 1u;
    int dbits = 1;
    while (dbits < 32 && (dspan >> dbits) != 0u) dbits++;
    const bool nine = (dbits + 8) / 9 < (dbits + 7) / 8;
    return BinningMode{dmin, dbits, dmin + dspan, nine ? 9 : 8, nullptr, drop_dead};
  }
};
inline DepthSortInput resident_depth_sort_input(char* bin, const GaussSortLayout& GS) { return depth_sort_input(bin, GS, DEPTH_KEY_BITS, BinningMode::RESIDENT_DIGIT_BITS); }

struct K1Targets {
  uint32_t *depth_keys = nullptr, *depth_vals = nullptr;
  uint2* ranges = nullptr;
  uint32_t extra_flags = 0u;
  uint32_t* depth_overflow = nullptr;
};

struct PerGaussianBwd {
  float* gacc = nullptr;
  bool depth = false;
  bool clean_gacc = false;
  const float* dz_in = nullptr;
  const segs_camera_grads* cam = nullptr;
  uint8_t* written = nullptr;
  bool packed = false;
};

struct Allocators { segs_alloc_fn geometry_alloc; void* geometry_ctx; segs_alloc_fn binning_alloc; void* binning_ctx; segs_alloc_fn image_alloc; void* image_ctx; };

enum GaccCleaning { MEMSET_PER_CALL, SELF_CLEAN };
struct BackwardInputs { const float* background; const int* radii; const float* dL_dpix; const segs_depth_grads* dgrad; const segs_camera_grads* cam; };

constexpr const Gaussians* K1_RAN_AT_PRODUCER = nullptr;
constexpr const segs_depth_outputs* NO_DEPTH_OUTPUTS = nullptr;
constexpr const segs_depth_grads* NO_DEPTH_GRADS = nullptr;
constexpr const segs_camera_grads* NO_CAMERA_GRADS = nullptr;
constexpr const float *NO_CAM_POS = nullptr, *NO_DL_DZ = nullptr;
constexpr int* NO_RADII = nullptr;

}
```

segs-slam_amd/csrc/gs_layout.h:

```cpp
#pragma once
#include <algorithm>
#include <cstddef>
#include <cstdint>

namespace segs {

constexpr int TILE_X = 16;
constexpr int TILE_Y = 16;
constexpr int NUM_CHANNELS = 3;

constexpr float LOG2E = 1.4426950408889634f;

constexpr int REC_DWORDS = 16;
enum RecField { REC_X = 0, REC_Y, REC_A2, REC_B2, REC_C2, REC_O, REC_R, REC_G, REC_B, REC_DEPTH, REC_RECT_MIN, REC_RECT_MAX, REC_CA, REC_CB, REC_CC };

struct BinInfo { uint32_t depth_bits, rect_min, rect_max, tiles_touched; };
constexpr uint32_t ID_BITS = 28;
constexpr uint32_t ID_MASK = (1u << ID_BITS) - 1u;
constexpr int MAX_GAUSSIANS = 1 << ID_BITS;

constexpr int GACC_DWORDS = 16;

constexpr size_t ALIGN = 256;
inline size_t align_up(size_t v, size_t a = ALIGN) { return (v + a - 1) / a * a; }

struct GeomLayout {
  size_t rec, bin, offsets, radii_internal, block_sums, clamped, num_rendered, gacc, touched, written, total;
  int P, nblocks;
};
inline GeomLayout geom_layout(int P) {
  GeomLayout g{};
  g.P = P;
  g.nblocks = (P + 255) / 256;
  size_t o = 0;
  g.rec = o;            o = align_up(o + (size_t)P * REC_DWORDS * 4);
  g.bin = o;            o = align_up(o + (size_t)P * sizeof(BinInfo));
  g.offsets = o;        o = align_up(o + (size_t)P * 4);
  g.radii_internal = o; o = align_up(o + (size_t)P * 4);
  g.block_sums = o;     o = align_up(o + (size_t)(g.nblocks + 1) * 4 * 3);
  g.clamped = o;        o = align_up(o + (size_t)P * 4);
  g.num_rendered = o;   o = align_up(o + 64);
  g.gacc = o;           o = align_up(o + (size_t)P * GACC_DWORDS * 4);
  g.touched = o;        o = align_up(o + (size_t)P * 4);
  g.written = o;        o = align_up(o + (size_t)P);
  g.total = o + ALIGN;
  return g;
}

struct ImageLayout {
  size_t ranges, final_T, n_contrib, total;
};
inline ImageLayout image_layout(int W, int H) {
  ImageLayout l{};
  const size_t tiles = (size_t)((W + TILE_X - 1) / TILE_X) * ((H + TILE_Y - 1) / TILE_Y);
  size_t o = 0;
  l.ranges = o;    o = align_up(o + tiles * 8);
  l.final_T = o;   o = align_up(o + (size_t)W * H * 4);
  l.n_contrib = o; o = align_up(o + (size_t)W * H * 4);
  l.total = o + ALIGN;
  return l;
}

#ifndef SEGS_SORT_ITEMS_PER_THREAD
#define SEGS_SORT_ITEMS_PER_THREAD 8
#endif
constexpr int SORT_ITEMS_PER_THREAD = SEGS_SORT_ITEMS_PER_THREAD;
constexpr int SORT_THREADS = 256;
constexpr int SORT_TILE = SORT_ITEMS_PER_THREAD * SORT_THREADS;
constexpr int PREFIX_ROWS_PER_WG = 8;
constexpr int EMIT_SLOTS_PER_WG = 512;
constexpr int SORT_COUNT_CHUNK_TILES = 4;
constexpr int RANGE_KEYS_PER_THREAD = 4;
constexpr int SORT_WIDE_DIGITS = 2048;
constexpr int SORT_WIDE_MAX_TILES = 1024;
constexpr int SORT_MAX_DIGITS = 512;

struct BinningLayout {
  size_t keys[2], vals[2], tile_prefix, chunk_hist, digit_totals, n_live, total;
  int nchunks;
  int R, nblocks;
};
inline BinningLayout binning_layout(int R) {
  BinningLayout b{};
  b.R = R;
  b.nblocks = (R + SORT_TILE - 1) / SORT_TILE;
  size_t o = 0;
  for (int i = 0; i < 2; i++) { b.keys[i] = o; o = align_up(o + (size_t)R * 8); }
  for (int i = 0; i < 2; i++) { b.vals[i] = o; o = align_up(o + (size_t)R * 4); }
  b.nchunks = b.nblocks;
  const size_t cols = (size_t)(b.nblocks > 0 ? b.nblocks : 1);
  const size_t matrix = std::max((size_t)SORT_MAX_DIGITS * cols, (size_t)SORT_WIDE_DIGITS * std::min(cols, (size_t)SORT_WIDE_MAX_TILES));
  b.tile_prefix = o;  o = align_up(o + matrix * 4);
  b.chunk_hist = o;   o = align_up(o + matrix * 4);
  b.digit_totals = o; o = align_up(o + SORT_WIDE_DIGITS * 4);
  b.n_live = o;       o = align_up(o + 4);
  b.total = o + ALIGN;
  return b;
}
struct GaussSortLayout {
  size_t base, block_sums, first_owner, total;
  BinningLayout inner;
};
inline GaussSortLayout gauss_sort_layout(int R, int P) {
  GaussSortLayout g{};
  g.inner = binning_layout(P);
  g.base = align_up(binning_layout(R).total);
  g.block_sums = g.base + align_up(g.inner.total);
  g.first_owner = g.block_sums + align_up((size_t)((P + 255) / 256 + 4) * 4);
  g.total = g.first_owner + align_up((size_t)(R / EMIT_SLOTS_PER_WG + 4) * 4) + ALIGN;
  return g;
}

inline char* align_ptr(char* p) { return (char*)(((uintptr_t)p + ALIGN - 1) / ALIGN * ALIGN); }
inline const char* align_ptr(const char* p) { return (const char*)(((uintptr_t)p + ALIGN - 1) / ALIGN * ALIGN); }

}
```

segs-slam_amd/csrc/kernels.h:

```cpp
#pragma once
#include <hip/hip_runtime.h>
#include <cstdint>
#include "gs_layout.h"

namespace segs {

int set_error(int code, const char* what);
int set_hip_error(hipError_t e, const char* where);


__global__ void preprocess_fwd_kernel(
    int P, const float* __restrict__ means3D, const float* __restrict__ scales, float mod,
    const float* __restrict__ rotations, const float* __restrict__ opacities, const float* __restrict__ colors,
    const float* __restrict__ cov3D_precomp, const float* __restrict__ viewmatrix, const float* __restrict__ projmatrix,
    int W, int H, float tan_fovx, float tan_fovy, float focal_x, float focal_y, uint32_t gx, uint32_t gy,
    int* __restrict__ radii, float* __restrict__ rec, BinInfo* __restrict__ bin, uint32_t* __restrict__ block_sums,
    uint32_t* __restrict__ depth_range, const float* __restrict__ shs, int D, int M, const float* __restrict__ cam_pos,
    uint32_t* __restrict__ clamped, uint32_t flags, uint32_t* __restrict__ depth_keys, uint32_t* __restrict__ depth_vals,
    uint2* __restrict__ ranges, int num_tiles, uint32_t* __restrict__ depth_overflow, uint32_t* __restrict__ touched_dense);
constexpr uint32_t DEPTH_KEY_MIN = 0x3E4CCCCDu;
constexpr int DEPTH_KEY_BITS = 27;

__global__ void visible_filter_kernel(
    int P, const float* __restrict__ means3D, const float* __restrict__ scales, float mod,
    const float* __restrict__ rotations, const float* __restrict__ cov3D_precomp,
    const float* __restrict__ viewmatrix, const float* __restrict__ projmatrix, int W, int H,
    float tan_fovx, float tan_fovy, float focal_x, float focal_y, uint32_t gx, uint32_t gy, int* __restrict__ radii,
    int log_scale_stride);

__global__ void mark_visible_kernel(int P, const float* __restrict__ means3D, const float* __restrict__ viewmatrix,
                                    uint8_t* __restrict__ present);

constexpr int CAM_SUMS = 24;
template <bool DEPTH, bool CAM>
__global__ void preprocess_bwd_kernel(
    int P, const float* __restrict__ means3D, const int* __restrict__ radii, const float* __restrict__ scales,
    const float* __restrict__ rotations, float mod, const float* __restrict__ cov3D_precomp,
    const float* __restrict__ view, const float* __restrict__ proj, float h_x, float h_y, float tan_fovx, float tan_fovy,
    float* __restrict__ gacc, float img_w, float img_h,
    float* __restrict__ dL_dmean2D, float* __restrict__ dL_dconic,
    float* __restrict__ dL_dopacity, float* __restrict__ dL_dcolor, float* __restrict__ dL_dmean3D,
    float* __restrict__ dL_dcov3D, float* __restrict__ dL_dscale, float* __restrict__ dL_drot, int clean_gacc,
    const float* __restrict__ dz_in, float* __restrict__ cam_partials, uint8_t* __restrict__ written);
template <bool DEPTH, bool CAM>
__global__ void preprocess_bwd_packed_kernel(
    int P, const float* __restrict__ means3D, const int* __restrict__ radii, const float* __restrict__ scales,
    const float* __restrict__ rotations, float mod, const float* __restrict__ cov3D_precomp,
    const float* __restrict__ view, const float* __restrict__ proj, float h_x, float h_y, float tan_fovx, float tan_fovy,
    float* __restrict__ gacc, float img_w, float img_h,
    float* __restrict__ dL_dmean2D, float* __restrict__ dL_dconic,
    float* __restrict__ dL_dopacity, float* __restrict__ dL_dcolor, float* __restrict__ dL_dmean3D,
    float* __restrict__ dL_dcov3D, float* __restrict__ dL_dscale, float* __restrict__ dL_drot,
    float* __restrict__ cam_partials, uint8_t* __restrict__ written);
__global__ void camera_grad_reduce_kernel(const float* __restrict__ partials, int nblocks, float* __restrict__ dL_dview,
                                          float* __restrict__ dL_dproj);
__global__ void sh_backward_kernel(int P, const float* __restrict__ means3D, const int* __restrict__ radii,
                                   const float* __restrict__ shs, int D, int M, const float* __restrict__ cam_pos,
                                   const uint32_t* __restrict__ clamped, const float* __restrict__ dL_dcolor,
                                   float* __restrict__ dL_dmean3D, float* __restrict__ dL_dsh);

__global__ void scan_block_sums_kernel(uint32_t* __restrict__ block_sums, int nblocks, const uint32_t* __restrict__ depth_range,
                                       uint32_t* __restrict__ total);
__global__ void ordered_offsets_kernel(int P, const uint32_t* __restrict__ block_sums, uint32_t* __restrict__ incl,
                                       uint32_t* __restrict__ total_out, const uint32_t* __restrict__ ng_dev,
                                       uint32_t* __restrict__ first_owner, uint32_t owner_entries);
__global__ void duplicate_with_keys_kernel(int P, int R, const float* __restrict__ rec,
                                           const uint32_t* __restrict__ order, const uint32_t* __restrict__ incl,
                                           uint32_t* __restrict__ keys, uint32_t* __restrict__ vals, uint32_t gx,
                                           const uint32_t* __restrict__ n_dev, int mark_dead, const uint32_t* __restrict__ ng_dev,
                                           const uint32_t* __restrict__ first_owner);
constexpr uint32_t RANGE_EMPTY_START = 0xFFFFFFFFu;
__global__ void normalize_ranges_kernel(int num_tiles, uint2* __restrict__ ranges);
constexpr uint32_t PREPROCESS_TIGHT_RECT = 0x80000000u;
constexpr uint32_t DEAD_KEY = 0xFFFFFFFFu;
template <typename K, int BITS>
__global__ void radix_count_kernel(const K* __restrict__ keys, int n, int shift, uint32_t dmin, int dbits,
                                   uint32_t* __restrict__ tile_prefix, uint32_t* __restrict__ chunk_hist, int nblocks, int nchunks,
                                   const uint32_t* __restrict__ n_dev, int drop_dead, int chunk_tiles, int nbits);
__global__ void radix_scan_kernel(uint32_t* __restrict__ block_hist, int nblocks, uint32_t* __restrict__ digit_totals);
template <typename K, int BITS, bool AUX>
__global__ void radix_scatter_kernel(const K* __restrict__ keys_in, const uint32_t* __restrict__ vals_in,
                                     K* __restrict__ keys_out, uint32_t* __restrict__ vals_out, int n, int shift,
                                     uint32_t dmin, int dbits, const uint32_t* __restrict__ tile_prefix, const uint32_t* __restrict__ chunk_prefix,
                                     const uint32_t* __restrict__ digit_totals, int nblocks, int nchunks,
                                     const uint32_t* __restrict__ n_dev, int drop_dead, uint32_t* __restrict__ n_live_out,
                                     const uint32_t* __restrict__ aux_in, uint32_t* __restrict__ aux_out, int nbits, int chunk_tiles, int pack_shift,
                                     uint2* __restrict__ ranges_out, uint32_t* __restrict__ status, uint32_t* __restrict__ status_mirror,
                                     int write_keys);
__global__ void identify_tile_ranges_kernel(int L, const uint32_t* __restrict__ keys, uint2* __restrict__ ranges,
                                            const uint32_t* __restrict__ n_dev, uint32_t* __restrict__ status,
                                            uint32_t* __restrict__ status_mirror, const uint32_t* __restrict__ n_live);

__global__ void render_fwd_kernel(const uint2* __restrict__ ranges, const uint32_t* __restrict__ point_list, int W, int H,
                                  const float* __restrict__ rec, const float* __restrict__ bg,
                                  float* __restrict__ final_T, uint32_t* __restrict__ n_contrib, float* __restrict__ out_color);
__global__ void render_bwd_kernel(const uint2* __restrict__ ranges, const uint32_t* __restrict__ point_list, int W, int H,
                                  const float* __restrict__ rec, const float* __restrict__ bg,
                                  const float* __restrict__ final_T, const uint32_t* __restrict__ n_contrib,
                                  const float* __restrict__ dL_dpix, float* __restrict__ gacc, uint32_t num_tiles,
                                  uint8_t* __restrict__ written);
__global__ void render_bwd_mfma_kernel(const uint2* __restrict__ ranges, const uint32_t* __restrict__ point_list, int W, int H,
                                       const float* __restrict__ rec, const float* __restrict__ bg,
                                       const float* __restrict__ final_T, const uint32_t* __restrict__ n_contrib,
                                       const float* __restrict__ dL_dpix, float* __restrict__ gacc, uint32_t num_tiles,
                                       uint8_t* __restrict__ written);
__global__ void render_fwd_depth_kernel(const uint2* __restrict__ ranges, const uint32_t* __restrict__ point_list, int W, int H,
                                        const float* __restrict__ rec, const float* __restrict__ bg,
                                        float* __restrict__ final_T, uint32_t* __restrict__ n_contrib, float* __restrict__ out_color,
                                        float* __restrict__ out_depth, float* __restrict__ out_alpha);
__global__ void render_bwd_depth_kernel(const uint2* __restrict__ ranges, const uint32_t* __restrict__ point_list, int W, int H,
                                        const float* __restrict__ rec, const float* __restrict__ bg,
                                        const float* __restrict__ final_T, const uint32_t* __restrict__ n_contrib,
                                        const float* __restrict__ dL_dpix, float* __restrict__ gacc, uint32_t num_tiles,
                                        const float* __restrict__ dL_ddepth, const float* __restrict__ dL_dalpha,
                                        uint8_t* __restrict__ written);

__global__ void unpack_geometry_kernel(int P, const float* __restrict__ rec, const BinInfo* __restrict__ bin,
                                       const int* __restrict__ radii, float* __restrict__ means2D,
                                       float* __restrict__ conic_opacity, float* __restrict__ depths,
                                       uint32_t* __restrict__ tiles_touched, float* __restrict__ rgb);

__global__ void rebuild_keys_kernel(int R, const uint32_t* __restrict__ tile_keys, const uint32_t* __restrict__ vals,
                                    const BinInfo* __restrict__ bin, uint64_t* __restrict__ keys64);
__global__ void make_depth_keys_kernel(int P, const BinInfo* __restrict__ bin, uint32_t dcull, uint32_t* __restrict__ keys,
                                       uint32_t* __restrict__ vals, uint2* __restrict__ ranges, int num_tiles);
__global__ void ordered_block_sums_kernel(int P, const uint32_t* touched, const uint32_t* __restrict__ order,
                                          uint32_t* __restrict__ block_sums, uint32_t* sorted_touched,
                                          const uint32_t* __restrict__ ng_dev, uint32_t* __restrict__ order_rw, int pack_shift);
__global__ void point_offsets_kernel(int P, const BinInfo* __restrict__ bin, uint32_t* __restrict__ offsets);
__global__ void strip_mask_kernel(int n, const uint32_t* __restrict__ vals, uint32_t* __restrict__ out);

}
```

segs-slam_amd/csrc/render.hip:

```cpp
#include <hip/hip_runtime.h>
#include <cstdint>
#include "gs_layout.h"
#include "kernels.h"

namespace segs {

__device__ __forceinline__ uint32_t xcd_tile(uint32_t wg, uint32_t num_tiles) {
  const uint32_t full = num_tiles & ~63u;
  if (wg >= full) return wg;
  const uint32_t xcd = wg & 7u, local = wg >> 3;
  return (local >> 3) * 64u + xcd * 8u + (local & 7u);
}

__device__ __forceinline__ float fast_exp2(float x) { return __builtin_amdgcn_exp2f(x); }
__device__ __forceinline__ float fast_rcp(float x) { return __builtin_amdgcn_rcpf(x); }
__device__ __forceinline__ uint32_t readlane_u32(uint32_t v, int lane) {
  return (uint32_t)__builtin_amdgcn_readlane((int)v, lane);
}


__device__ __forceinline__ float rl(float v, int lane) {
  return __int_as_float(__builtin_amdgcn_readlane(__float_as_int(v), lane));
}

__device__ __forceinline__ void wave_lds_fence() { asm volatile("" ::: "memory"); }

struct Compacted { uint32_t val; uint32_t pos; int n; };
template <bool REVERSE>
__device__ __forceinline__ Compacted compact_chunk(uint32_t v, uint32_t qbit, int lane) {
  const bool rel = (v & qbit) != 0u;
  const uint64_t m = __ballot(rel);
  const int n = __popcll(m);
  const int below = (int)__builtin_amdgcn_mbcnt_hi((uint32_t)(m >> 32), __builtin_amdgcn_mbcnt_lo((uint32_t)m, 0u));
  const int rank = REVERSE ? (n - 1 - below) : below;
  const int dest = rel ? rank : n + (lane - below);
  Compacted c;
  c.val = (uint32_t)__builtin_amdgcn_ds_permute(dest << 2, (int)v);
  c.pos = (uint32_t)__builtin_amdgcn_ds_permute(dest << 2, lane);
  c.n = n;
  return c;
}

constexpr int FWD_REC = 12;

template <bool DEPTH>
__device__ __forceinline__ void load_rec_tail(const float4* p, float& rb, float& rz) {
  if (DEPTH) { const float2 t = reinterpret_cast<const float2*>(p)[4]; rb = t.x; rz = t.y; }
  else rb = reinterpret_cast<const float*>(p)[8];
}

template <bool DEPTH>
__device__ __forceinline__ void render_fwd_body(
    const uint2* __restrict__ ranges, const uint32_t* __restrict__ point_list, int W, int H,
    const float* __restrict__ rec, const float* __restrict__ bg, float* __restrict__ final_T,
    uint32_t* __restrict__ n_contrib, float* __restrict__ out_color, float* __restrict__ out_depth,
    float* __restrict__ out_alpha) {
  __shared__ float4 s_rec[4][64][FWD_REC / 4];
  const uint32_t tiles_x = (W + TILE_X - 1) / TILE_X;
  const uint32_t tile = xcd_tile(blockIdx.x, gridDim.x);
  const uint32_t tile_x = tile % tiles_x, tile_y = tile / tiles_x;
  const int lane = threadIdx.x & 63;
  const int wv = __builtin_amdgcn_readfirstlane(threadIdx.x >> 6);
  const uint32_t px = tile_x * TILE_X + (wv & 1) * 8 + (lane & 7);
  const uint32_t py = tile_y * TILE_Y + (wv >> 1) * 8 + (lane >> 3);
  const bool inside = px < (uint32_t)W && py < (uint32_t)H;
  const float pxf = (float)px, pyf = (float)py;
  const uint32_t qbit = 1u << (ID_BITS + wv);

  const uint2 range = ranges[tile];
  bool live = inside;
  float T = 1.0f, C0 = 0.f, C1 = 0.f, C2 = 0.f, Dz = 0.f;
  uint32_t last = 0u;

  uint32_t v_nxt, v_nn = 0u;
  Compacted cc;
  float4 r0, r1; float rb, rz = 0.f;
  {
    const uint32_t i0 = range.x + lane, i1 = range.x + 64 + lane;
    const uint32_t v0 = i0 < range.y ? point_list[i0] : 0u;
    v_nxt = i1 < range.y ? point_list[i1] : 0u;
    cc = compact_chunk<false>(v0, qbit, lane);
    r0 = make_float4(0.f, 0.f, 0.f, 0.f); r1 = r0; rb = 0.f;
    if (lane < cc.n) {
      const float4* p = reinterpret_cast<const float4*>(rec + (size_t)(cc.val & ID_MASK) * REC_DWORDS);
      r0 = p[0]; r1 = p[1]; load_rec_tail<DEPTH>(p, rb, rz);
    }
  }
  bool alive = true;
  for (uint32_t base = range.x; base < range.y && alive; base += 64) {
    const int n = __builtin_amdgcn_readfirstlane(cc.n);
    const int n4 = (n + 3) & ~3;
    if (lane < n4) {
      const bool real = lane < n;
      s_rec[wv][lane][0] = real ? r0 : make_float4(0.f, 0.f, 0.f, 0.f);
      s_rec[wv][lane][1] = real ? r1 : make_float4(0.f, 0.f, 0.f, 0.f);
      s_rec[wv][lane][2] = make_float4(real ? rb : 0.f, __uint_as_float(base - range.x + cc.pos + 1u), (DEPTH && real) ? rz : 0.f, 0.f);
    }
    wave_lds_fence();
    {
      const uint32_t i2 = base + 128 + lane;
      v_nn = i2 < range.y ? point_list[i2] : 0u;
      cc = compact_chunk<false>(v_nxt, qbit, lane);
      if (lane < cc.n) {
        const float4* p = reinterpret_cast<const float4*>(rec + (size_t)(cc.val & ID_MASK) * REC_DWORDS);
        r0 = p[0]; r1 = p[1]; load_rec_tail<DEPTH>(p, rb, rz);
      }
      v_nxt = v_nn;
    }
    for (int k0 = 0; k0 < n4 && alive; k0 += 4) {
#pragma unroll
      for (int u = 0; u < 4; u++) {
        const int k = k0 + u;
        const float4 q0 = s_rec[wv][k][0], q1 = s_rec[wv][k][1];
        const float2 q2 = *reinterpret_cast<const float2*>(&s_rec[wv][k][2]);
        const float qz = DEPTH ? s_rec[wv][k][2].z : 0.f;
        const float dx = q0.x - pxf, dy = q0.y - pyf;
        const float power2 = dx * (q0.z * dx + q0.w * dy) + (q1.x * dy) * dy;
        const float alpha = fminf(0.99f, q1.y * fast_exp2(power2));
        bool take = power2 <= 0.0f && alpha >= 1.0f / 255.0f && live;
        const float ae = take ? alpha : 0.f;
        float w = ae * T;
        float test_T = T - w;
        const bool stop = test_T < 0.0001f;
        if (__ballot(stop) != 0ull) {
          live = live && !stop;
          take = take && !stop;
          w = stop ? 0.f : w;
          test_T = stop ? T : test_T;
        }
        T = test_T;
        C0 += q1.z * w; C1 += q1.w * w; C2 += q2.x * w;
        if (DEPTH) Dz += qz * w;
        last = take ? __float_as_uint(q2.y) : last;
      }
      alive = __ballot(live) != 0ull;
    }
  }
  if (inside) {
    const size_t pix_id = (size_t)W * py + px;
    const size_t HW = (size_t)H * W;
    final_T[pix_id] = T;
    n_contrib[pix_id] = last;
    out_color[pix_id] = C0 + T * bg[0];
    out_color[HW + pix_id] = C1 + T * bg[1];
    out_color[2 * HW + pix_id] = C2 + T * bg[2];
    if (DEPTH) {
      if (out_depth) out_depth[pix_id] = Dz;
      if (out_alpha) out_alpha[pix_id] = 1.0f - T;
    }
  }
}

__global__ void __launch_bounds__(256) render_fwd_kernel(
    const uint2* __restrict__ ranges, const uint32_t* __restrict__ point_list, int W, int H,
    const float* __restrict__ rec, const float* __restrict__ bg, float* __restrict__ final_T,
    uint32_t* __restrict__ n_contrib, float* __restrict__ out_color) {
  render_fwd_body<false>(ranges, point_list, W, H, rec, bg, final_T, n_contrib, out_color, nullptr, nullptr);
}
__global__ void __launch_bounds__(256) render_fwd_depth_kernel(
    const uint2* __restrict__ ranges, const uint32_t* __restrict__ point_list, int W, int H,
    const float* __restrict__ rec, const float* __restrict__ bg, float* __restrict__ final_T,
    uint32_t* __restrict__ n_contrib, float* __restrict__ out_color, float* __restrict__ out_depth,
    float* __restrict__ out_alpha) {
  render_fwd_body<true>(ranges, point_list, W, H, rec, bg, final_T, n_contrib, out_color, out_depth, out_alpha);
}

__device__ __forceinline__ float fold32(float a, float b) {
  auto r = __builtin_amdgcn_permlane32_swap(__float_as_uint(a), __float_as_uint(b), false, false);
  return __uint_as_float(r[0]) + __uint_as_float(r[1]);
}
__device__ __forceinline__ float fold16(float x, float y) {
  auto r = __builtin_amdgcn_permlane16_swap(__float_as_uint(x), __float_as_uint(y), false, false);
  return __uint_as_float(r[0]) + __uint_as_float(r[1]);
}
__device__ __forceinline__ float fold_rows4(float a, float b, float c, float d) {
  return fold16(fold32(a, b), fold32(c, d));
}

template <int I>
__device__ __forceinline__ void fmac_row_bcast(float& acc, float v, float a) {
  asm("v_fmac_f32_dpp %0, %1, %2 row_newbcast:%3 row_mask:0xf bank_mask:0xf bound_ctrl:1" : "+v"(acc) : "v"(v), "v"(a), "n"(I));
}
constexpr int BW_SLOTS = 16;
constexpr int BW_STRIDE = 65;
struct BwdLds {
  float4 rec[BW_SLOTS][3];
  float2 wa[BW_SLOTS][BW_STRIDE];
};


template <bool USE_BG, bool DEPTH>
__device__ __forceinline__ void pixel_role(BwdLds& L, int nb, int lane, float pxf, float pyf, uint32_t last_contributor,
                                           float dp0, float dp1, float dp2, float dpz, float T_final, float bg_dot_dpixel,
                                           float& T, float& accd) {
#ifndef PIX_UNROLL
#define PIX_UNROLL 4
#endif
#pragma unroll PIX_UNROLL
  for (int sl = 0; sl < nb; sl++) {
    const float4 q0 = L.rec[sl][0], q1 = L.rec[sl][1];
    const float2 q2 = *reinterpret_cast<const float2*>(&L.rec[sl][2]);
    const float qz = DEPTH ? L.rec[sl][2].w : 0.f;
    const float dx = q0.x - pxf, dy = q0.y - pyf;
    const float power2 = dx * (q0.z * dx + q0.w * dy) + (q1.x * dy) * dy;
#if defined(SEGS_MEASURE) && defined(ABLATE_NO_TRANS)
    const float ar = q1.y * (power2 * 0.001f + 1.0f);
#else
    const float ar = q1.y * fast_exp2(power2);
#endif
    const bool ok = __float_as_uint(q2.y) < last_contributor && power2 <= 0.0f && ar >= 1.0f / 255.0f;
    const float aw = ok ? ar : 0.f;
    const float ae = fminf(0.99f, aw);
#if defined(SEGS_MEASURE) && defined(ABLATE_NO_TRANS)
    const float rinv = 1.f + ae;
#else
    const float rinv = fast_rcp(1.f - ae);
#endif
    T = T * rinv;
    const float diff = (DEPTH ? (q1.z * dp0 + q1.w * dp1 + q2.x * dp2 + qz * dpz) : (q1.z * dp0 + q1.w * dp1 + q2.x * dp2)) - accd;
    float dL_dalpha = diff * T;
    if (USE_BG) dL_dalpha += (-T_final * rinv) * bg_dot_dpixel;
    accd += ae * diff;
    L.wa[sl][lane] = make_float2(aw * dL_dalpha , ae * T );
  }
}

typedef float f32x4 __attribute__((ext_vector_type(4)));

template <bool MFMA, bool DEPTH>
__device__ __forceinline__ void render_bwd_body(
    const uint2* __restrict__ ranges, const uint32_t* __restrict__ point_list, int W, int H,
    const float* __restrict__ rec, const float* __restrict__ bg, const float* __restrict__ final_T,
    const uint32_t* __restrict__ n_contrib, const float* __restrict__ dL_dpix, float* __restrict__ gacc, uint32_t num_tiles,
    const float* __restrict__ dL_ddepth, const float* __restrict__ dL_dalpha, uint8_t* __restrict__ written) {
  static_assert(!(MFMA && DEPTH), "the depth form of the tile backward is the VALU form");
  __shared__ BwdLds lds_one;
  const uint32_t tiles_x = (W + TILE_X - 1) / TILE_X;
  const uint32_t xcd = blockIdx.x & 7u, local = blockIdx.x >> 3;
  const uint32_t v = ((local >> 2) << 3) | xcd;
  if (v >= num_tiles) return;
  const uint32_t tile = xcd_tile(v, num_tiles);
  const uint32_t tile_x = tile % tiles_x, tile_y = tile / tiles_x;
  const int lane = threadIdx.x & 63;
  const int wv = __builtin_amdgcn_readfirstlane((int)(local & 3u));
  BwdLds& L = lds_one;
  const uint32_t qx0 = tile_x * TILE_X + (wv & 1) * 8, qy0 = tile_y * TILE_Y + (wv >> 1) * 8;
  const uint32_t px = qx0 + (lane & 7), py = qy0 + (lane >> 3);
  const bool inside = px < (uint32_t)W && py < (uint32_t)H;
  const float pxf = (float)px, pyf = (float)py;
  const size_t pix_id = (size_t)W * py + px;
  const size_t HW = (size_t)H * W;
  const uint32_t qbit = 1u << (ID_BITS + wv);

  const uint2 range = ranges[tile];
  const float T_final = inside ? final_T[pix_id] : 0.f;
  const uint32_t last_contributor = inside ? n_contrib[pix_id] : 0u;
  float dp0 = 0.f, dp1 = 0.f, dp2 = 0.f;
  if (inside) { dp0 = dL_dpix[pix_id]; dp1 = dL_dpix[HW + pix_id]; dp2 = dL_dpix[2 * HW + pix_id]; }
  float dpz = 0.f, dpa = 0.f;
  if (DEPTH && inside) { dpz = dL_ddepth ? dL_ddepth[pix_id] : 0.f; dpa = dL_dalpha ? dL_dalpha[pix_id] : 0.f; }
  const float bg_dot_dpixel = DEPTH ? (bg[0] * dp0 + bg[1] * dp1 + bg[2] * dp2) - dpa : bg[0] * dp0 + bg[1] * dp1 + bg[2] * dp2;
  const bool use_bg = __ballot(bg_dot_dpixel != 0.f) != 0ull;

  uint32_t wave_last = last_contributor;
#pragma unroll
  for (int off = 32; off > 0; off >>= 1) wave_last = max(wave_last, (uint32_t)__shfl_xor((int)wave_last, off, 64));
  wave_last = __builtin_amdgcn_readfirstlane(wave_last);
  if (wave_last == 0u) return;

  float T = T_final, accd = 0.f;

  const int gs = lane & 15, part = lane >> 4;
  const float pyl0 = (float)(part * 2), pyl1 = pyl0 + 1.0f;
  const float qx0f = (float)qx0, qy0f = (float)qy0;

  float bmono[16], bcol[16];
  if (MFMA) {
    float* dps = reinterpret_cast<float*>(&L.wa[0][0]);
    dps[lane] = dp0; dps[64 + lane] = dp1; dps[128 + lane] = dp2;
    wave_lds_fence();
    const float j1 = gs == 1 ? 1.f : 0.f, j3 = gs == 3 ? 1.f : 0.f, j4 = gs == 4 ? 1.f : 0.f;
    const bool colour = gs >= 6 && gs < 9;
    const int crow = colour ? (gs - 6) * 64 + part * 16 : 0;
#pragma unroll
    for (int h = 0; h < 2; h++) {
      const float y = (float)(2 * part + h) - 3.5f;
      const float c0 = gs == 0 ? 1.f : gs == 2 ? y : gs == 5 ? y * y : 0.f;
      const float c1 = j1 + j4 * y;
#pragma unroll
      for (int c = 0; c < 8; c++) {
        const float x = (float)c - 3.5f;
        bmono[8 * h + c] = c0 + x * (c1 + x * j3);
      }
    }
#pragma unroll
    for (int t = 0; t < 16; t++) { const float v = dps[crow + t]; bcol[t] = colour ? v : 0.f; }
    wave_lds_fence();
  }

  const int32_t cfirst = (int32_t)((wave_last - 1u) & ~63u);
  uint32_t v_nxt = 0u;
  Compacted cc;
  float4 r0, r1; float rb, rz = 0.f;
  {
    const uint32_t p0 = (uint32_t)cfirst + lane;
    const uint32_t v0 = p0 < wave_last ? point_list[range.x + p0] : 0u;
    if (cfirst >= 64) v_nxt = point_list[range.x + (uint32_t)(cfirst - 64) + lane];
    cc = compact_chunk<true>(v0, qbit, lane);
    r0 = make_float4(0.f, 0.f, 0.f, 0.f); r1 = r0; rb = 0.f;
    if (lane < cc.n) {
      const float4* p = reinterpret_cast<const float4*>(rec + (size_t)(cc.val & ID_MASK) * REC_DWORDS);
      r0 = p[0]; r1 = p[1]; load_rec_tail<DEPTH>(p, rb, rz);
    }
  }
  float (*mom)[12] = reinterpret_cast<float (*)[12]>(&L.wa[0][0]);
  int fill = 0;
  for (int32_t cbase = cfirst;; cbase -= 64) {
    const bool tail = cbase < 0;
    const int n = tail ? 0 : __builtin_amdgcn_readfirstlane(cc.n);
    const float4 c0 = r0, c1 = r1;
    const float4 c2 = make_float4(rb, __uint_as_float((uint32_t)cbase + cc.pos), __uint_as_float(cc.val & ID_MASK), DEPTH ? rz : 0.f);
    if (cbase >= 64) {
      uint32_t v_nn = 0u;
      if (cbase >= 128) v_nn = point_list[range.x + (uint32_t)(cbase - 128) + lane];
      cc = compact_chunk<true>(v_nxt, qbit, lane);
      if (lane < cc.n) {
        const float4* p = reinterpret_cast<const float4*>(rec + (size_t)(cc.val & ID_MASK) * REC_DWORDS);
        r0 = p[0]; r1 = p[1]; load_rec_tail<DEPTH>(p, rb, rz);
      }
      v_nxt = v_nn;
    }
    int taken = 0;
    do {
      const int take = min(BW_SLOTS - fill, n - taken);
      if (lane >= taken && lane < taken + take) {
        const int s = fill + lane - taken;
        L.rec[s][0] = c0; L.rec[s][1] = c1; L.rec[s][2] = c2;
      }
      fill += take; taken += take;
      if (fill < BW_SLOTS && !(tail && fill > 0)) continue;
      const int nb = fill;
      fill = 0;
      wave_lds_fence();
      if (use_bg) pixel_role<true, DEPTH>(L, nb, lane, pxf, pyf, last_contributor, dp0, dp1, dp2, dpz, T_final, bg_dot_dpixel, T, accd);
      else pixel_role<false, DEPTH>(L, nb, lane, pxf, pyf, last_contributor, dp0, dp1, dp2, dpz, T_final, bg_dot_dpixel, T, accd);
      wave_lds_fence();
#if defined(SEGS_MEASURE) && defined(ABLATE_NO_GAUSS_ROLE)
      continue;
#endif
      const float2 gxy = *reinterpret_cast<const float2*>(&L.rec[gs][0]);
      const float gxr = gxy.x - qx0f, gyr = gxy.y - qy0f;
      float cx, cy;
      if (MFMA) {
        cx = 3.5f; cy = 3.5f;
        f32x4 dw = {0.f, 0.f, 0.f, 0.f}, da = {0.f, 0.f, 0.f, 0.f};
        const float2* warow = &L.wa[gs][part * 16];
#pragma unroll
        for (int t = 0; t < 16; t++) {
          const float2 wa_t = warow[t];
#ifdef SEGS_MFMA_ONE_CHAIN
          dw = __builtin_amdgcn_mfma_f32_16x16x4f32(wa_t.x, bmono[t], dw, 0, 0, 0);
          dw = __builtin_amdgcn_mfma_f32_16x16x4f32(wa_t.y, bcol[t], dw, 0, 0, 0);
#else
          dw = __builtin_amdgcn_mfma_f32_16x16x4f32(wa_t.x, bmono[t], dw, 0, 0, 0);
          da = __builtin_amdgcn_mfma_f32_16x16x4f32(wa_t.y, bcol[t], da, 0, 0, 0);
#endif
        }
        if (gs < 9) {
#pragma unroll
          for (int r = 0; r < 4; r++) mom[4 * part + r][gs] = dw[r] + da[r];
        }
      } else {
      cx = fminf(7.f, fmaxf(0.f, rintf(gxr))); cy = fminf(7.f, fmaxf(0.f, rintf(gyr)));
      float px8[8], px8q[8];
#pragma unroll
      for (int c = 0; c < 8; c++) { px8[c] = (float)c - cx; px8q[c] = px8[c] * px8[c]; }
      const float pyc0 = pyl0 - cy, pyc1 = pyl1 - cy;
      float S0, S1x, S1y, Sxx, Sxy, Syy, Sr = 0.f, Sg = 0.f, Sb = 0.f, Sz = 0.f;
      {
        float R0[2] = {0.f, 0.f}, R1[2] = {0.f, 0.f}, R2[2] = {0.f, 0.f};
        const float2* warow = &L.wa[gs][part * 16];
#define GAUSS_STEP(i)                                                                         \
        {                                                                                     \
          const float2 wa_i = warow[i];                                                       \
          const float w = wa_i.x, a = wa_i.y;                                                 \
          R0[(i) >> 3] += w; R1[(i) >> 3] += w * px8[(i) & 7]; R2[(i) >> 3] += w * px8q[(i) & 7]; \
          fmac_row_bcast<(i)>(Sr, dp0, a); fmac_row_bcast<(i)>(Sg, dp1, a); fmac_row_bcast<(i)>(Sb, dp2, a); \
          if (DEPTH) fmac_row_bcast<(i)>(Sz, dpz, a);                                         \
        }
        GAUSS_STEP(0) GAUSS_STEP(1) GAUSS_STEP(2) GAUSS_STEP(3) GAUSS_STEP(4) GAUSS_STEP(5) GAUSS_STEP(6) GAUSS_STEP(7)
        GAUSS_STEP(8) GAUSS_STEP(9) GAUSS_STEP(10) GAUSS_STEP(11) GAUSS_STEP(12) GAUSS_STEP(13) GAUSS_STEP(14) GAUSS_STEP(15)
#undef GAUSS_STEP
        S0 = R0[0] + R0[1]; S1x = R1[0] + R1[1]; Sxx = R2[0] + R2[1];
        S1y = pyc0 * R0[0] + pyc1 * R0[1];
        Sxy = pyc0 * R1[0] + pyc1 * R1[1];
        Syy = (pyc0 * pyc0) * R0[0] + (pyc1 * pyc1) * R0[1];
      }
      const float g1 = fold_rows4(S0, S1y, S1x, Sxx);
      const float g2 = fold_rows4(Sxy, Sr, Syy, Sg);
      if (DEPTH) {
        const float g3 = fold_rows4(Sb, Sz, Sb, Sz);
        mom[gs][part] = g1;
        mom[gs][4 + part] = g2;
        if ((part & 1) == 0) mom[gs][8 + (part >> 1)] = g3;
      } else {
      const float g3 = fold_rows4(Sb, Sb, Sb, Sb);
      mom[gs][part] = g1;
      mom[gs][4 + part] = g2;
      if (part == 0) mom[gs][8] = g3;
      }
      }
      wave_lds_fence();
      uint32_t id_gs;
      {
        const float4 m0 = *reinterpret_cast<const float4*>(&mom[gs][0]);
        const float4 m1 = *reinterpret_cast<const float4*>(&mom[gs][4]);
        const float m8 = mom[gs][8];
        const float hx = gxr - cx, hy = gyr - cy;
        const float Mx = hx * m0.x - m0.y, My = hy * m0.x - m0.z;
        const float Mxx = hx * (hx * m0.x - 2.f * m0.y) + m0.w;
        const float Mxy = hx * (hy * m0.x - m0.z) - hy * m0.y + m1.x;
        const float Myy = hy * (hy * m0.x - 2.f * m0.z) + m1.y;
        wave_lds_fence();
        const float inv_o = fast_rcp(reinterpret_cast<const float*>(&L.rec[gs][1])[1]);
        id_gs = __float_as_uint(reinterpret_cast<const float*>(&L.rec[gs][2])[2]);
        wave_lds_fence();
        if (part == 0) {
          *reinterpret_cast<float4*>(&mom[gs][0]) = make_float4(Mx, My, Mxx, Mxy);
          *reinterpret_cast<float4*>(&mom[gs][4]) = make_float4(Myy, m0.x * inv_o, m1.z, m1.w);
          mom[gs][8] = m8;
        }
      }
      wave_lds_fence();
#pragma unroll
      for (int j = 0; j < 4; j++) {
        const int slot = 4 * j + part;
        if (slot < nb && gs < (DEPTH ? 10 : 9)) {
          const uint32_t id = __float_as_uint(reinterpret_cast<const float*>(&L.rec[slot][2])[2]);
#if !(defined(SEGS_MEASURE) && defined(ABLATE_NO_ATOMICS))
          atomicAdd(gacc + (size_t)id * GACC_DWORDS + gs, mom[slot][gs]);
#endif
        }
      }
      if (written && lane < nb) {
        uint32_t one;
        asm volatile("v_mov_b32 %0, 1" : "=v"(one));
        written[id_gs] = (uint8_t)one;
      }
      wave_lds_fence();
    } while (taken < n);
    if (tail) break;
  }
}

__global__ void __launch_bounds__(64) render_bwd_kernel(
    const uint2* __restrict__ ranges, const uint32_t* __restrict__ point_list, int W, int H,
    const float* __restrict__ rec, const float* __restrict__ bg, const float* __restrict__ final_T,
    const uint32_t* __restrict__ n_contrib, const float* __restrict__ dL_dpix, float* __restrict__ gacc, uint32_t num_tiles,
    uint8_t* __restrict__ written) {
  render_bwd_body<false, false>(ranges, point_list, W, H, rec, bg, final_T, n_contrib, dL_dpix, gacc, num_tiles, nullptr, nullptr, written);
}
__global__ void __launch_bounds__(64) render_bwd_mfma_kernel(
    const uint2* __restrict__ ranges, const uint32_t* __restrict__ point_list, int W, int H,
    const float* __restrict__ rec, const float* __restrict__ bg, const float* __restrict__ final_T,
    const uint32_t* __restrict__ n_contrib, const float* __restrict__ dL_dpix, float* __restrict__ gacc, uint32_t num_tiles,
    uint8_t* __restrict__ written) {
  render_bwd_body<true, false>(ranges, point_list, W, H, rec, bg, final_T, n_contrib, dL_dpix, gacc, num_tiles, nullptr, nullptr, written);
}
__global__ void __launch_bounds__(64) render_bwd_depth_kernel(
    const uint2* __restrict__ ranges, const uint32_t* __restrict__ point_list, int W, int H,
    const float* __restrict__ rec, const float* __restrict__ bg, const float* __restrict__ final_T,
    const uint32_t* __restrict__ n_contrib, const float* __restrict__ dL_dpix, float* __restrict__ gacc, uint32_t num_tiles,
    const float* __restrict__ dL_ddepth, const float* __restrict__ dL_dalpha, uint8_t* __restrict__ written) {
  render_bwd_body<false, true>(ranges, point_list, W, H, rec, bg, final_T, n_contrib, dL_dpix, gacc, num_tiles, dL_ddepth, dL_dalpha, written);
}

}
```

Baseline: 1100 iters/s.

## Record per-wave contributing-splat walk lists in forward and replay them in backward

The forward render kernel now records, per wave quadrant, which list positions had any live contributing pixel (via ballot masks) and writes them into a new walk buffer placed after the binning sort scratch, with per-tile counts in the image buffer. The backward kernel, when self-cleaning is on and the new flag is not set, replays these compact lists in reverse instead of rescanning and compacting the full per-tile point list. This skips backward work on splats that contributed to no pixel in a wave, at the cost of extra forward writes, larger binning and image buffers, and more kernel variants.

```diff
diff --git a/include/segs_raster.h b/include/segs_raster.h
--- a/include/segs_raster.h
+++ b/include/segs_raster.h
@@ -26,6 +26,7 @@
 #define SEGS_RASTER_MFMA_MOMENTS 64u
 #define SEGS_RASTER_NO_WRITTEN_BYTES 128u
 #define SEGS_RASTER_UNPACKED_BACKWARD 256u
+#define SEGS_RASTER_NO_WALK_LISTS 512u
 uint32_t segs_raster_set_flags(uint32_t flags);
 
 uint32_t* segs_raster_set_status_mirror(uint32_t* host_mapped_status);
@@ -84,6 +85,9 @@
 int segs_debug_instance_values(const char* binning_buffer, int R, uint32_t* values , void* stream);
 int segs_debug_unpack_image(const char* image_buffer, int width, int height, uint32_t* ranges ,
                             float* final_T , uint32_t* n_contrib , void* stream);
+
+size_t segs_resident_walk_offset(int P, int capacity);
+size_t segs_image_walk_count_offset(int width, int height);
 
 #define SEGS_GEOMETRY_REGIONS 10
 int segs_debug_geometry_layout(int P, size_t* offset_and_bytes , int regions);
diff --git a/segs-slam_amd/_capi.py b/segs-slam_amd/_capi.py
--- a/segs-slam_amd/_capi.py
+++ b/segs-slam_amd/_capi.py
@@ -110,6 +110,8 @@
     "segs_debug_instance_values": (_i, [_vp, _i, _vp, _vp]),
     "segs_debug_unpack_binning": (_i, [_vp, _vp, _i, _i, _i, _i, _vp, _vp, _vp]),
     "segs_debug_unpack_image": (_i, [_vp, _i, _i, _vp, _vp, _vp, _vp]),
+    "segs_resident_walk_offset": (_sz, [_i, _i]),
+    "segs_image_walk_count_offset": (_sz, [_i, _i]),
     "segs_debug_preprocess_backward": (_i, [_i, _i, _i, _vp, _vp, _vp, _f, _vp, _vp, _vp, _vp, _f, _f, _vp, _vp, _vp,
                                              _vp, _vp, _vp, _vp]),
     "segs_debug_preprocess_backward_camera": (_i, [_i, _i, _i, _vp, _vp, _vp, _f, _vp, _vp, _vp, _vp, _f, _f, _vp, _vp, _vp,
diff --git a/segs-slam_amd/csrc/capi.hip b/segs-slam_amd/csrc/capi.hip
--- a/segs-slam_amd/csrc/capi.hip
+++ b/segs-slam_amd/csrc/capi.hip
@@ -167,6 +167,7 @@
 }
 
 bool drop_dead_instances() { return (g_flags & SEGS_RASTER_KEEP_DEAD_INSTANCES) == 0u; }
+bool walk_lists() { return (g_flags & SEGS_RASTER_NO_WALK_LISTS) == 0u; }
 uint32_t resident_k1_flags() { return drop_dead_instances() ? PREPROCESS_TIGHT_RECT : 0u; }
 
 int run_preprocess(const Geom& G, const Gaussians& g, const View& V, int* radii, const K1Targets& k1, hipStream_t st) {
@@ -260,9 +261,16 @@
 }
 
 int launch_render_fwd(const Scratch& S, const View& V, const float* background, float* out_color, const segs_depth_outputs* dout,
-                      hipStream_t st) {
+                      bool walk, hipStream_t st) {
   PROF(K_RENDER_FWD);
-  if (dout && (dout->depth || dout->alpha))
+  const bool depth = dout && (dout->depth || dout->alpha);
+  if (walk && depth)
+    render_fwd_depth_walk_kernel<<<V.tiles, 256, 0, st>>>(S.ranges(), S.point_list(), V.width, V.height, S.G.rec(), background, S.final_T(),
+                                                          S.n_contrib(), out_color, dout->depth, dout->alpha, S.walk(), S.walk_count());
+  else if (walk)
+    render_fwd_walk_kernel<<<V.tiles, 256, 0, st>>>(S.ranges(), S.point_list(), V.width, V.height, S.G.rec(), background, S.final_T(),
+                                                    S.n_contrib(), out_color, S.walk(), S.walk_count());
+  else if (depth)
     render_fwd_depth_kernel<<<V.tiles, 256, 0, st>>>(S.ranges(), S.point_list(), V.width, V.height, S.G.rec(), background, S.final_T(),
                                                      S.n_contrib(), out_color, dout->depth, dout->alpha);
   else
@@ -273,17 +281,33 @@
 }
 
 int launch_render_bwd(const Scratch& S, const View& V, const float* background, const float* dL_dpix, const segs_depth_grads* dgrad,
-                      uint8_t* written, hipStream_t st) {
+                      uint8_t* written, bool walk, hipStream_t st) {
   PROF(K_RENDER_BWD);
   const uint32_t grid = (V.tiles + 7) / 8 * 32;
-  if (dgrad && (dgrad->dL_ddepth || dgrad->dL_dalpha)) {
+  const bool depth = dgrad && (dgrad->dL_ddepth || dgrad->dL_dalpha);
+  if (walk && depth) {
+    render_bwd_depth_walk_kernel<<<grid, 64, 0, st>>>(S.ranges(), S.point_list(), V.width, V.height, S.G.rec(), background, S.final_T(),
+                                                      S.n_contrib(), dL_dpix, S.G.gacc(), V.tiles, dgrad->dL_ddepth, dgrad->dL_dalpha, written,
+                                                      S.walk(), S.walk_count());
+    LAUNCH_TRY("render_bwd_depth_walk_kernel");
+    return SEGS_OK;
+  }
+  if (depth) {
     render_bwd_depth_kernel<<<grid, 64, 0, st>>>(S.ranges(), S.point_list(), V.width, V.height, S.G.rec(), background, S.final_T(),
                                                  S.n_contrib(), dL_dpix, S.G.gacc(), V.tiles, dgrad->dL_ddepth, dgrad->dL_dalpha, written);
     LAUNCH_TRY("render_bwd_depth_kernel");
     return SEGS_OK;
   }
   static const bool mfma_env = [] { const char* e = getenv("SEGS_RENDER_BWD_MFMA"); return e && e[0] == '1'; }();
-  ((mfma_env || (g_flags & SEGS_RASTER_MFMA_MOMENTS)) ? render_bwd_mfma_kernel : render_bwd_kernel)<<<grid, 64, 0, st>>>(
+  const bool mfma = mfma_env || (g_flags & SEGS_RASTER_MFMA_MOMENTS);
+  if (walk) {
+    (mfma ? render_bwd_mfma_walk_kernel : render_bwd_walk_kernel)<<<grid, 64, 0, st>>>(
+        S.ranges(), S.point_list(), V.width, V.height, S.G.rec(), background, S.final_T(), S.n_contrib(), dL_dpix, S.G.gacc(), V.tiles, written,
+        S.walk(), S.walk_count());
+    LAUNCH_TRY("render_bwd_walk_kernel");
+    return SEGS_OK;
+  }
+  (mfma ? render_bwd_mfma_kernel : render_bwd_kernel)<<<grid, 64, 0, st>>>(
       S.ranges(), S.point_list(), V.width, V.height, S.G.rec(), background, S.final_T(), S.n_contrib(), dL_dpix, S.G.gacc(), V.tiles, written);
   LAUNCH_TRY("render_bwd_kernel");
   return SEGS_OK;
@@ -395,7 +419,7 @@
                                        : BinningMode::exact_range(hdr[1], hdr[2], tight);
     if (int rc = run_binning(S, V, mode, st)) return rc;
   }
-  if (int rc = launch_render_fwd(S, V, background, out_color, dout, st)) return rc;
+  if (int rc = launch_render_fwd(S, V, background, out_color, dout, false, st)) return rc;
   *num_rendered = R;
   return SEGS_OK;
 }
@@ -425,7 +449,7 @@
     if (int rc = run_preprocess(S.G, *k1, V, radii ? radii : S.G.radii_internal(), t, st)) return rc;
   }
   if (int rc = run_binning(S, V, BinningMode::resident_keys(keys.keys, drop_dead_instances()), st)) return rc;
-  return launch_render_fwd(S, V, background, out_color, dout, st);
+  return launch_render_fwd(S, V, background, out_color, dout, walk_lists(), st);
 }
 
 int rasterize_backward(const Gaussians& g, const View& V, const ScratchBuffers& B, const BackwardInputs& in, const GradOutputs& o,
@@ -458,7 +482,7 @@
   m.written = (self_clean && !(g_flags & SEGS_RASTER_NO_WRITTEN_BYTES)) ? G.written() : nullptr;
   m.packed = m.written && !(g_flags & SEGS_RASTER_UNPACKED_BACKWARD);
   if (R > 0)
-    if (int rc = launch_render_bwd(S, V, in.background, in.dL_dpix, in.dgrad, m.written, st)) return rc;
+    if (int rc = launch_render_bwd(S, V, in.background, in.dL_dpix, in.dgrad, m.written, self_clean && walk_lists(), st)) return rc;
   { PROF(K_PREPROCESS_BWD);
   if (int rc = launch_preprocess_bwd(g, V, radii, o, m, st)) return rc;
   }
@@ -770,7 +794,9 @@
 }
 
 
-size_t segs_resident_binning_bytes(int P, int capacity) { return gauss_sort_layout(capacity < 0 ? 0 : capacity, P < 0 ? 0 : P).total; }
+size_t segs_resident_binning_bytes(int P, int capacity) { return walk_layout(capacity < 0 ? 0 : capacity, P < 0 ? 0 : P).total; }
+size_t segs_resident_walk_offset(int P, int capacity) { return walk_layout(capacity < 0 ? 0 : capacity, P < 0 ? 0 : P).walk; }
+size_t segs_image_walk_count_offset(int width, int height) { return image_layout(width, height).walk_count; }
 
 int segs_rasterize_forward_resident(char* geom_buffer, char* binning_buffer, char* image_buffer, int capacity, int geom_rows, int P, int D, int M,
                                     const float* background, int width, int height, const float* means3D, const float* shs,
diff --git a/segs-slam_amd/csrc/capi_args.h b/segs-slam_amd/csrc/capi_args.h
--- a/segs-slam_amd/csrc/capi_args.h
+++ b/segs-slam_amd/csrc/capi_args.h
@@ -85,6 +85,8 @@
   const uint32_t* point_list() const { return (const uint32_t*)(bin + BL.vals[0]); }
   float* final_T() const { return (float*)(img + IL.final_T); }
   uint32_t* n_contrib() const { return (uint32_t*)(img + IL.n_contrib); }
+  uint32_t* walk() const { return (uint32_t*)(bin + align_up(GS.total)); }
+  uint32_t* walk_count() const { return (uint32_t*)(img + IL.walk_count); }
 };
 inline Scratch carve(const ScratchBuffers& B, int P, const View& V, uint32_t* status) {
   return Scratch{geom_at(B.geom_buffer, P, B.geom_rows), align_ptr(B.image_buffer), align_ptr(B.binning_buffer), image_layout(V.width, V.height),
diff --git a/segs-slam_amd/csrc/gs_layout.h b/segs-slam_amd/csrc/gs_layout.h
--- a/segs-slam_amd/csrc/gs_layout.h
+++ b/segs-slam_amd/csrc/gs_layout.h
@@ -48,7 +48,7 @@
 }
 
 struct ImageLayout {
-  size_t ranges, final_T, n_contrib, total;
+  size_t ranges, final_T, n_contrib, walk_count, total;
 };
 inline ImageLayout image_layout(int W, int H) {
   ImageLayout l{};
@@ -57,6 +57,7 @@
   l.ranges = o;    o = align_up(o + tiles * 8);
   l.final_T = o;   o = align_up(o + (size_t)W * H * 4);
   l.n_contrib = o; o = align_up(o + (size_t)W * H * 4);
+  l.walk_count = o; o = align_up(o + tiles * 4 * 4);
   l.total = o + ALIGN;
   return l;
 }
@@ -111,6 +112,14 @@
   return g;
 }
 
+struct WalkLayout { size_t walk, total; };
+inline WalkLayout walk_layout(int R, int P) {
+  WalkLayout w{};
+  w.walk = align_up(gauss_sort_layout(R, P).total);
+  w.total = w.walk + align_up((size_t)R * 4 * 4) + ALIGN;
+  return w;
+}
+
 inline char* align_ptr(char* p) { return (char*)(((uintptr_t)p + ALIGN - 1) / ALIGN * ALIGN); }
 inline const char* align_ptr(const char* p) { return (const char*)(((uintptr_t)p + ALIGN - 1) / ALIGN * ALIGN); }
 
diff --git a/segs-slam_amd/csrc/kernels.h b/segs-slam_amd/csrc/kernels.h
--- a/segs-slam_amd/csrc/kernels.h
+++ b/segs-slam_amd/csrc/kernels.h
@@ -115,6 +115,35 @@
                                         const float* __restrict__ dL_ddepth, const float* __restrict__ dL_dalpha,
                                         uint8_t* __restrict__ written);
 
+__global__ void render_fwd_walk_kernel(const uint2* __restrict__ ranges, const uint32_t* __restrict__ point_list, int W, int H,
+                                       const float* __restrict__ rec, const float* __restrict__ bg,
+                                       float* __restrict__ final_T, uint32_t* __restrict__ n_contrib, float* __restrict__ out_color,
+                                       uint32_t* __restrict__ walk, uint32_t* __restrict__ walk_count);
+__global__ void render_fwd_depth_walk_kernel(const uint2* __restrict__ ranges, const uint32_t* __restrict__ point_list, int W, int H,
+                                             const float* __restrict__ rec, const float* __restrict__ bg,
+                                             float* __restrict__ final_T, uint32_t* __restrict__ n_contrib, float* __restrict__ out_color,
+                                             float* __restrict__ out_depth, float* __restrict__ out_alpha,
+                                             uint32_t* __restrict__ walk, uint32_t* __restrict__ walk_count);
+__global__ void render_bwd_walk_kernel(const uint2* __restrict__ ranges, const uint32_t* __restrict__ point_list, int W, int H,
+                                       const float* __restrict__ rec, const float* __restrict__ bg,
+                                       const float* __restrict__ final_T, const uint32_t* __restrict__ n_contrib,
+                                       const float* __restrict__ dL_dpix, float* __restrict__ gacc, uint32_t num_tiles,
+                                       uint8_t* __restrict__ written, const uint32_t* __restrict__ walk,
+                                       const uint32_t* __restrict__ walk_count);
+__global__ void render_bwd_mfma_walk_kernel(const uint2* __restrict__ ranges, const uint32_t* __restrict__ point_list, int W, int H,
+                                            const float* __restrict__ rec, const float* __restrict__ bg,
+                                            const float* __restrict__ final_T, const uint32_t* __restrict__ n_contrib,
+                                            const float* __restrict__ dL_dpix, float* __restrict__ gacc, uint32_t num_tiles,
+                                            uint8_t* __restrict__ written, const uint32_t* __restrict__ walk,
+                                            const uint32_t* __restrict__ walk_count);
+__global__ void render_bwd_depth_walk_kernel(const uint2* __restrict__ ranges, const uint32_t* __restrict__ point_list, int W, int H,
+                                             const float* __restrict__ rec, const float* __restrict__ bg,
+                                             const float* __restrict__ final_T, const uint32_t* __restrict__ n_contrib,
+                                             const float* __restrict__ dL_dpix, float* __restrict__ gacc, uint32_t num_tiles,
+                                             const float* __restrict__ dL_ddepth, const float* __restrict__ dL_dalpha,
+                                             uint8_t* __restrict__ written, const uint32_t* __restrict__ walk,
+                                             const uint32_t* __restrict__ walk_count);
+
 __global__ void unpack_geometry_kernel(int P, const float* __restrict__ rec, const BinInfo* __restrict__ bin,
                                        const int* __restrict__ radii, float* __restrict__ means2D,
                                        float* __restrict__ conic_opacity, float* __restrict__ depths,
diff --git a/segs-slam_amd/csrc/render.hip b/segs-slam_amd/csrc/render.hip
--- a/segs-slam_amd/csrc/render.hip
+++ b/segs-slam_amd/csrc/render.hip
@@ -41,6 +41,11 @@
   return c;
 }
 
+__device__ __forceinline__ uint64_t lane_mask(bool p) { return __builtin_amdgcn_ballot_w64(p); }
+__device__ __forceinline__ void shift_in_any(uint32_t& acc, uint64_t mask) {
+  asm("s_cmp_lg_u64 %1, 0\n\ts_addc_u32 %0, %0, %0" : "+s"(acc) : "s"(mask) : "scc");
+}
+
 constexpr int FWD_REC = 12;
 
 template <bool DEPTH>
@@ -49,12 +54,12 @@
   else rb = reinterpret_cast<const float*>(p)[8];
 }
 
-template <bool DEPTH>
+template <bool DEPTH, bool WALK>
 __device__ __forceinline__ void render_fwd_body(
     const uint2* __restrict__ ranges, const uint32_t* __restrict__ point_list, int W, int H,
     const float* __restrict__ rec, const float* __restrict__ bg, float* __restrict__ final_T,
     uint32_t* __restrict__ n_contrib, float* __restrict__ out_color, float* __restrict__ out_depth,
-    float* __restrict__ out_alpha) {
+    float* __restrict__ out_alpha, uint32_t* __restrict__ walk, uint32_t* __restrict__ walk_count) {
   __shared__ float4 s_rec[4][64][FWD_REC / 4];
   const uint32_t tiles_x = (W + TILE_X - 1) / TILE_X;
   const uint32_t tile = xcd_tile(blockIdx.x, gridDim.x);
@@ -69,6 +74,7 @@
 
   const uint2 range = ranges[tile];
   bool live = inside;
+  uint64_t live_m = lane_mask(inside);
   float T = 1.0f, C0 = 0.f, C1 = 0.f, C2 = 0.f, Dz = 0.f;
   uint32_t last = 0u;
 
@@ -87,6 +93,8 @@
     }
   }
   bool alive = true;
+  uint32_t* const wl = walk + ((size_t)range.x * 4u + (size_t)wv * (range.y - range.x));
+  uint32_t wcnt = 0u;
   for (uint32_t base = range.x; base < range.y && alive; base += 64) {
     const int n = __builtin_amdgcn_readfirstlane(cc.n);
     const int n4 = (n + 3) & ~3;
@@ -107,35 +115,63 @@
       }
       v_nxt = v_nn;
     }
-    for (int k0 = 0; k0 < n4 && alive; k0 += 4) {
-#pragma unroll
-      for (int u = 0; u < 4; u++) {
-        const int k = k0 + u;
-        const float4 q0 = s_rec[wv][k][0], q1 = s_rec[wv][k][1];
-        const float2 q2 = *reinterpret_cast<const float2*>(&s_rec[wv][k][2]);
-        const float qz = DEPTH ? s_rec[wv][k][2].z : 0.f;
-        const float dx = q0.x - pxf, dy = q0.y - pyf;
-        const float power2 = dx * (q0.z * dx + q0.w * dy) + (q1.x * dy) * dy;
-        const float alpha = fminf(0.99f, q1.y * fast_exp2(power2));
-        bool take = power2 <= 0.0f && alpha >= 1.0f / 255.0f && live;
-        const float ae = take ? alpha : 0.f;
-        float w = ae * T;
-        float test_T = T - w;
-        const bool stop = test_T < 0.0001f;
-        if (__ballot(stop) != 0ull) {
-          live = live && !stop;
-          take = take && !stop;
-          w = stop ? 0.f : w;
-          test_T = stop ? T : test_T;
-        }
-        T = test_T;
-        C0 += q1.z * w; C1 += q1.w * w; C2 += q2.x * w;
-        if (DEPTH) Dz += qz * w;
-        last = take ? __float_as_uint(q2.y) : last;
-      }
-      alive = __ballot(live) != 0ull;
-    }
-  }
+#define FWD_GROUP(acc)                                                                                                     \
+      {                                                                                                                    \
+        _Pragma("unroll") for (int u = 0; u < 4; u++) {                                                                    \
+          const int k = k0 + u;                                                                                            \
+          const float4 q0 = s_rec[wv][k][0], q1 = s_rec[wv][k][1];                                                         \
+          const float2 q2 = *reinterpret_cast<const float2*>(&s_rec[wv][k][2]);                                            \
+          const float qz = DEPTH ? s_rec[wv][k][2].z : 0.f;                                                                \
+          const float dx = q0.x - pxf, dy = q0.y - pyf;                                                                    \
+          const float power2 = dx * (q0.z * dx + q0.w * dy) + (q1.x * dy) * dy;                         \
+          const float alpha = fminf(0.99f, q1.y * fast_exp2(power2));                                                      \
+                          \
+          bool take = power2 <= 0.0f && alpha >= 1.0f / 255.0f && live;                                                    \
+                                                 \
+          uint64_t take_m = 0ull;                                                                                          \
+          if (WALK) take_m = lane_mask(power2 <= 0.0f) & lane_mask(alpha >= 1.0f / 255.0f) & live_m;                       \
+          const float ae = take ? alpha : 0.f;                                                                             \
+          float w = ae * T;                                                                                                \
+          float test_T = T - w;                                                                                            \
+          const bool stop = test_T < 0.0001f;                                                      \
+          const uint64_t stop_m = WALK ? lane_mask(stop) : 0ull;                        \
+                                    \
+          if (WALK ? stop_m != 0ull : __ballot(stop) != 0ull) {                                                            \
+            live = live && !stop;                                                                                          \
+            take = take && !stop;                                                                                          \
+            w = stop ? 0.f : w;                                                                                            \
+            test_T = stop ? T : test_T;                                                                                    \
+            if (WALK) { live_m &= ~stop_m; take_m &= ~stop_m; }                                                            \
+          }                                                                                                                \
+          T = test_T;                                                                                                      \
+          C0 += q1.z * w; C1 += q1.w * w; C2 += q2.x * w;                                                                  \
+          if (DEPTH) Dz += qz * w;                                                                                         \
+          last = take ? __float_as_uint(q2.y) : last;                                                                      \
+          if (WALK) shift_in_any(acc, take_m);                 \
+        }                                                                                                                  \
+                                       \
+        alive = WALK ? live_m != 0ull : __ballot(live) != 0ull;                                                            \
+      }
+    uint32_t acc_lo = 0u, acc_hi = 0u;
+    const int split = WALK ? min(n4, 32) : n4;
+    int k0 = 0;
+    for (; k0 < split && alive; k0 += 4) FWD_GROUP(acc_lo)
+    if (WALK) {
+      const int e_lo = k0;
+      for (k0 = 32; k0 < n4 && alive; k0 += 4) FWD_GROUP(acc_hi)
+      const int e_hi = k0 - 32;
+      const uint32_t taken_lo = e_lo ? __builtin_bitreverse32(acc_lo) >> (32 - e_lo) : 0u;
+      const uint32_t taken_hi = e_hi ? __builtin_bitreverse32(acc_hi) >> (32 - e_hi) : 0u;
+      const uint32_t pos1 = __float_as_uint(s_rec[wv][lane][2].y);
+      if (((lane < 32 ? taken_lo : taken_hi) >> (lane & 31)) & 1u) {
+        const uint32_t at = __builtin_amdgcn_mbcnt_hi(taken_hi, __builtin_amdgcn_mbcnt_lo(taken_lo, 0u));
+        wl[wcnt + at] = pos1 - 1u;
+      }
+      wcnt += (uint32_t)(__popc(taken_lo) + __popc(taken_hi));
+    }
+#undef FWD_GROUP
+  }
+  if (WALK && lane == 0) walk_count[tile * 4u + (uint32_t)wv] = wcnt;
   if (inside) {
     const size_t pix_id = (size_t)W * py + px;
     const size_t HW = (size_t)H * W;
@@ -155,14 +191,27 @@
     const uint2* __restrict__ ranges, const uint32_t* __restrict__ point_list, int W, int H,
     const float* __restrict__ rec, const float* __restrict__ bg, float* __restrict__ final_T,
     uint32_t* __restrict__ n_contrib, float* __restrict__ out_color) {
-  render_fwd_body<false>(ranges, point_list, W, H, rec, bg, final_T, n_contrib, out_color, nullptr, nullptr);
+  render_fwd_body<false, false>(ranges, point_list, W, H, rec, bg, final_T, n_contrib, out_color, nullptr, nullptr, nullptr, nullptr);
 }
 __global__ void __launch_bounds__(256) render_fwd_depth_kernel(
     const uint2* __restrict__ ranges, const uint32_t* __restrict__ point_list, int W, int H,
     const float* __restrict__ rec, const float* __restrict__ bg, float* __restrict__ final_T,
     uint32_t* __restrict__ n_contrib, float* __restrict__ out_color, float* __restrict__ out_depth,
     float* __restrict__ out_alpha) {
-  render_fwd_body<true>(ranges, point_list, W, H, rec, bg, final_T, n_contrib, out_color, out_depth, out_alpha);
+  render_fwd_body<true, false>(ranges, point_list, W, H, rec, bg, final_T, n_contrib, out_color, out_depth, out_alpha, nullptr, nullptr);
+}
+__global__ void __launch_bounds__(256) render_fwd_walk_kernel(
+    const uint2* __restrict__ ranges, const uint32_t* __restrict__ point_list, int W, int H,
+    const float* __restrict__ rec, const float* __restrict__ bg, float* __restrict__ final_T,
+    uint32_t* __restrict__ n_contrib, float* __restrict__ out_color, uint32_t* __restrict__ walk, uint32_t* __restrict__ walk_count) {
+  render_fwd_body<false, true>(ranges, point_list, W, H, rec, bg, final_T, n_contrib, out_color, nullptr, nullptr, walk, walk_count);
+}
+__global__ void __launch_bounds__(256) render_fwd_depth_walk_kernel(
+    const uint2* __restrict__ ranges, const uint32_t* __restrict__ point_list, int W, int H,
+    const float* __restrict__ rec, const float* __restrict__ bg, float* __restrict__ final_T,
+    uint32_t* __restrict__ n_contrib, float* __restrict__ out_color, float* __restrict__ out_depth,
+    float* __restrict__ out_alpha, uint32_t* __restrict__ walk, uint32_t* __restrict__ walk_count) {
+  render_fwd_body<true, true>(ranges, point_list, W, H, rec, bg, final_T, n_contrib, out_color, out_depth, out_alpha, walk, walk_count);
 }
 
 __device__ __forceinline__ float fold32(float a, float b) {
@@ -227,12 +276,13 @@
 
 typedef float f32x4 __attribute__((ext_vector_type(4)));
 
-template <bool MFMA, bool DEPTH>
+template <bool MFMA, bool DEPTH, bool WALK>
 __device__ __forceinline__ void render_bwd_body(
     const uint2* __restrict__ ranges, const uint32_t* __restrict__ point_list, int W, int H,
     const float* __restrict__ rec, const float* __restrict__ bg, const float* __restrict__ final_T,
     const uint32_t* __restrict__ n_contrib, const float* __restrict__ dL_dpix, float* __restrict__ gacc, uint32_t num_tiles,
-    const float* __restrict__ dL_ddepth, const float* __restrict__ dL_dalpha, uint8_t* __restrict__ written) {
+    const float* __restrict__ dL_ddepth, const float* __restrict__ dL_dalpha, uint8_t* __restrict__ written,
+    const uint32_t* __restrict__ walk, const uint32_t* __restrict__ walk_count) {
   static_assert(!(MFMA && DEPTH), "the depth form of the tile backward is the VALU form");
   __shared__ BwdLds lds_one;
   const uint32_t tiles_x = (W + TILE_X - 1) / TILE_X;
@@ -262,11 +312,19 @@
   const float bg_dot_dpixel = DEPTH ? (bg[0] * dp0 + bg[1] * dp1 + bg[2] * dp2) - dpa : bg[0] * dp0 + bg[1] * dp1 + bg[2] * dp2;
   const bool use_bg = __ballot(bg_dot_dpixel != 0.f) != 0ull;
 
-  uint32_t wave_last = last_contributor;
-#pragma unroll
-  for (int off = 32; off > 0; off >>= 1) wave_last = max(wave_last, (uint32_t)__shfl_xor((int)wave_last, off, 64));
-  wave_last = __builtin_amdgcn_readfirstlane(wave_last);
-  if (wave_last == 0u) return;
+  uint32_t wave_last = 0u, count = 0u;
+  const uint32_t list_len = range.y - range.x;
+  if (WALK) {
+    if (range.x >= range.y) return;
+    count = min((uint32_t)__builtin_amdgcn_readfirstlane((int)walk_count[tile * 4u + (uint32_t)wv]), list_len);
+    if (count == 0u) return;
+  } else {
+    wave_last = last_contributor;
+#pragma unroll
+    for (int off = 32; off > 0; off >>= 1) wave_last = max(wave_last, (uint32_t)__shfl_xor((int)wave_last, off, 64));
+    wave_last = __builtin_amdgcn_readfirstlane(wave_last);
+    if (wave_last == 0u) return;
+  }
 
   float T = T_final, accd = 0.f;
 
@@ -298,55 +356,14 @@
     wave_lds_fence();
   }
 
-  const int32_t cfirst = (int32_t)((wave_last - 1u) & ~63u);
-  uint32_t v_nxt = 0u;
-  Compacted cc;
-  float4 r0, r1; float rb, rz = 0.f;
-  {
-    const uint32_t p0 = (uint32_t)cfirst + lane;
-    const uint32_t v0 = p0 < wave_last ? point_list[range.x + p0] : 0u;
-    if (cfirst >= 64) v_nxt = point_list[range.x + (uint32_t)(cfirst - 64) + lane];
-    cc = compact_chunk<true>(v0, qbit, lane);
-    r0 = make_float4(0.f, 0.f, 0.f, 0.f); r1 = r0; rb = 0.f;
-    if (lane < cc.n) {
-      const float4* p = reinterpret_cast<const float4*>(rec + (size_t)(cc.val & ID_MASK) * REC_DWORDS);
-      r0 = p[0]; r1 = p[1]; load_rec_tail<DEPTH>(p, rb, rz);
-    }
-  }
   float (*mom)[12] = reinterpret_cast<float (*)[12]>(&L.wa[0][0]);
-  int fill = 0;
-  for (int32_t cbase = cfirst;; cbase -= 64) {
-    const bool tail = cbase < 0;
-    const int n = tail ? 0 : __builtin_amdgcn_readfirstlane(cc.n);
-    const float4 c0 = r0, c1 = r1;
-    const float4 c2 = make_float4(rb, __uint_as_float((uint32_t)cbase + cc.pos), __uint_as_float(cc.val & ID_MASK), DEPTH ? rz : 0.f);
-    if (cbase >= 64) {
-      uint32_t v_nn = 0u;
-      if (cbase >= 128) v_nn = point_list[range.x + (uint32_t)(cbase - 128) + lane];
-      cc = compact_chunk<true>(v_nxt, qbit, lane);
-      if (lane < cc.n) {
-        const float4* p = reinterpret_cast<const float4*>(rec + (size_t)(cc.val & ID_MASK) * REC_DWORDS);
-        r0 = p[0]; r1 = p[1]; load_rec_tail<DEPTH>(p, rb, rz);
-      }
-      v_nxt = v_nn;
-    }
-    int taken = 0;
-    do {
-      const int take = min(BW_SLOTS - fill, n - taken);
-      if (lane >= taken && lane < taken + take) {
-        const int s = fill + lane - taken;
-        L.rec[s][0] = c0; L.rec[s][1] = c1; L.rec[s][2] = c2;
-      }
-      fill += take; taken += take;
-      if (fill < BW_SLOTS && !(tail && fill > 0)) continue;
-      const int nb = fill;
-      fill = 0;
+  auto run_batch = [&](const int nb) {
       wave_lds_fence();
       if (use_bg) pixel_role<true, DEPTH>(L, nb, lane, pxf, pyf, last_contributor, dp0, dp1, dp2, dpz, T_final, bg_dot_dpixel, T, accd);
       else pixel_role<false, DEPTH>(L, nb, lane, pxf, pyf, last_contributor, dp0, dp1, dp2, dpz, T_final, bg_dot_dpixel, T, accd);
       wave_lds_fence();
 #if defined(SEGS_MEASURE) && defined(ABLATE_NO_GAUSS_ROLE)
-      continue;
+      return;
 #endif
       const float2 gxy = *reinterpret_cast<const float2*>(&L.rec[gs][0]);
       const float gxr = gxy.x - qx0f, gyr = gxy.y - qy0f;
@@ -448,8 +465,90 @@
         written[id_gs] = (uint8_t)one;
       }
       wave_lds_fence();
+  };
+
+  float4 r0, r1; float rb, rz = 0.f;
+  if constexpr (WALK) {
+    const uint32_t* const wl = walk + ((size_t)range.x * 4u + (size_t)wv * list_len);
+    int32_t top = (int32_t)count - 1;
+    const auto load_pos = [&](int32_t t) { const int32_t i = t - lane; return i >= 0 ? min(wl[i], list_len - 1u) : 0u; };
+    const auto load_val = [&](int32_t t, uint32_t pos) { return t - lane >= 0 ? point_list[range.x + pos] & ID_MASK : 0u; };
+    uint32_t pos_c = load_pos(top), pos_n = load_pos(top - 64), pos_nn = load_pos(top - 128);
+    uint32_t val_c = load_val(top, pos_c), val_n = load_val(top - 64, pos_n);
+    r0 = make_float4(0.f, 0.f, 0.f, 0.f); r1 = r0; rb = 0.f;
+    if (top - lane >= 0) {
+      const float4* p = reinterpret_cast<const float4*>(rec + (size_t)val_c * REC_DWORDS);
+      r0 = p[0]; r1 = p[1]; load_rec_tail<DEPTH>(p, rb, rz);
+    }
+    for (;; top -= 64) {
+      const int n = min(64, top + 1);
+      const float4 c0 = r0, c1 = r1;
+      const float4 c2 = make_float4(rb, __uint_as_float(pos_c), __uint_as_float(val_c), DEPTH ? rz : 0.f);
+      if (top >= 64) {
+        pos_c = pos_n; val_c = val_n;
+        if (top - 64 - lane >= 0) {
+          const float4* p = reinterpret_cast<const float4*>(rec + (size_t)val_c * REC_DWORDS);
+          r0 = p[0]; r1 = p[1]; load_rec_tail<DEPTH>(p, rb, rz);
+        }
+        pos_n = pos_nn;
+        val_n = load_val(top - 128, pos_n);
+        pos_nn = load_pos(top - 192);
+      }
+#pragma unroll 1
+      for (int j = 0; j < 64 / BW_SLOTS; j++) {
+        const int nb = min(BW_SLOTS, n - j * BW_SLOTS);
+        if (nb <= 0) break;
+        if ((lane >> 4) == j && (lane & 15) < nb) { L.rec[lane & 15][0] = c0; L.rec[lane & 15][1] = c1; L.rec[lane & 15][2] = c2; }
+        run_batch(nb);
+      }
+      if (top < 64) break;
+    }
+  } else {
+  const int32_t cfirst = (int32_t)((wave_last - 1u) & ~63u);
+  uint32_t v_nxt = 0u;
+  Compacted cc;
+  {
+    const uint32_t p0 = (uint32_t)cfirst + lane;
+    const uint32_t v0 = p0 < wave_last ? point_list[range.x + p0] : 0u;
+    if (cfirst >= 64) v_nxt = point_list[range.x + (uint32_t)(cfirst - 64) + lane];
+    cc = compact_chunk<true>(v0, qbit, lane);
+    r0 = make_float4(0.f, 0.f, 0.f, 0.f); r1 = r0; rb = 0.f;
+    if (lane < cc.n) {
+      const float4* p = reinterpret_cast<const float4*>(rec + (size_t)(cc.val & ID_MASK) * REC_DWORDS);
+      r0 = p[0]; r1 = p[1]; load_rec_tail<DEPTH>(p, rb, rz);
+    }
+  }
+  int fill = 0;
+  for (int32_t cbase = cfirst;; cbase -= 64) {
+    const bool tail = cbase < 0;
+    const int n = tail ? 0 : __builtin_amdgcn_readfirstlane(cc.n);
+    const float4 c0 = r0, c1 = r1;
+    const float4 c2 = make_float4(rb, __uint_as_float((uint32_t)cbase + cc.pos), __uint_as_float(cc.val & ID_MASK), DEPTH ? rz : 0.f);
+    if (cbase >= 64) {
+      uint32_t v_nn = 0u;
+      if (cbase >= 128) v_nn = point_list[range.x + (uint32_t)(cbase - 128) + lane];
+      cc = compact_chunk<true>(v_nxt, qbit, lane);
+      if (lane < cc.n) {
+        const float4* p = reinterpret_cast<const float4*>(rec + (size_t)(cc.val & ID_MASK) * REC_DWORDS);
+        r0 = p[0]; r1 = p[1]; load_rec_tail<DEPTH>(p, rb, rz);
+      }
+      v_nxt = v_nn;
+    }
+    int taken = 0;
+    do {
+      const int take = min(BW_SLOTS - fill, n - taken);
+      if (lane >= taken && lane < taken + take) {
+        const int s = fill + lane - taken;
+        L.rec[s][0] = c0; L.rec[s][1] = c1; L.rec[s][2] = c2;
+      }
+      fill += take; taken += take;
+      if (fill < BW_SLOTS && !(tail && fill > 0)) continue;
+      const int nb = fill;
+      fill = 0;
+      run_batch(nb);
     } while (taken < n);
     if (tail) break;
+  }
   }
 }
 
@@ -458,21 +557,44 @@
     const float* __restrict__ rec, const float* __restrict__ bg, const float* __restrict__ final_T,
     const uint32_t* __restrict__ n_contrib, const float* __restrict__ dL_dpix, float* __restrict__ gacc, uint32_t num_tiles,
     uint8_t* __restrict__ written) {
-  render_bwd_body<false, false>(ranges, point_list, W, H, rec, bg, final_T, n_contrib, dL_dpix, gacc, num_tiles, nullptr, nullptr, written);
+  render_bwd_body<false, false, false>(ranges, point_list, W, H, rec, bg, final_T, n_contrib, dL_dpix, gacc, num_tiles, nullptr, nullptr, written, nullptr, nullptr);
 }
 __global__ void __launch_bounds__(64) render_bwd_mfma_kernel(
     const uint2* __restrict__ ranges, const uint32_t* __restrict__ point_list, int W, int H,
     const float* __restrict__ rec, const float* __restrict__ bg, const float* __restrict__ final_T,
     const uint32_t* __restrict__ n_contrib, const float* __restrict__ dL_dpix, float* __restrict__ gacc, uint32_t num_tiles,
     uint8_t* __restrict__ written) {
-  render_bwd_body<true, false>(ranges, point_list, W, H, rec, bg, final_T, n_contrib, dL_dpix, gacc, num_tiles, nullptr, nullptr, written);
+  render_bwd_body<true, false, false>(ranges, point_list, W, H, rec, bg, final_T, n_contrib, dL_dpix, gacc, num_tiles, nullptr, nullptr, written, nullptr, nullptr);
 }
 __global__ void __launch_bounds__(64) render_bwd_depth_kernel(
     const uint2* __restrict__ ranges, const uint32_t* __restrict__ point_list, int W, int H,
     const float* __restrict__ rec, const float* __restrict__ bg, const float* __restrict__ final_T,
     const uint32_t* __restrict__ n_contrib, const float* __restrict__ dL_dpix, float* __restrict__ gacc, uint32_t num_tiles,
     const float* __restrict__ dL_ddepth, const float* __restrict__ dL_dalpha, uint8_t* __restrict__ written) {
-  render_bwd_body<false, true>(ranges, point_list, W, H, rec, bg, final_T, n_contrib, dL_dpix, gacc, num_tiles, dL_ddepth, dL_dalpha, written);
-}
-
-}
+  render_bwd_body<false, true, false>(ranges, point_list, W, H, rec, bg, final_T, n_contrib, dL_dpix, gacc, num_tiles, dL_ddepth, dL_dalpha, written, nullptr, nullptr);
+}
+
+__global__ void __launch_bounds__(64) render_bwd_walk_kernel(
+    const uint2* __restrict__ ranges, const uint32_t* __restrict__ point_list, int W, int H,
+    const float* __restrict__ rec, const float* __restrict__ bg, const float* __restrict__ final_T,
+    const uint32_t* __restrict__ n_contrib, const float* __restrict__ dL_dpix, float* __restrict__ gacc, uint32_t num_tiles,
+    uint8_t* __restrict__ written, const uint32_t* __restrict__ walk, const uint32_t* __restrict__ walk_count) {
+  render_bwd_body<false, false, true>(ranges, point_list, W, H, rec, bg, final_T, n_contrib, dL_dpix, gacc, num_tiles, nullptr, nullptr, written, walk, walk_count);
+}
+__global__ void __launch_bounds__(64) render_bwd_mfma_walk_kernel(
+    const uint2* __restrict__ ranges, const uint32_t* __restrict__ point_list, int W, int H,
+    const float* __restrict__ rec, const float* __restrict__ bg, const float* __restrict__ final_T,
+    const uint32_t* __restrict__ n_contrib, const float* __restrict__ dL_dpix, float* __restrict__ gacc, uint32_t num_tiles,
+    uint8_t* __restrict__ written, const uint32_t* __restrict__ walk, const uint32_t* __restrict__ walk_count) {
+  render_bwd_body<true, false, true>(ranges, point_list, W, H, rec, bg, final_T, n_contrib, dL_dpix, gacc, num_tiles, nullptr, nullptr, written, walk, walk_count);
+}
+__global__ void __launch_bounds__(64) render_bwd_depth_walk_kernel(
+    const uint2* __restrict__ ranges, const uint32_t* __restrict__ point_list, int W, int H,
+    const float* __restrict__ rec, const float* __restrict__ bg, const float* __restrict__ final_T,
+    const uint32_t* __restrict__ n_contrib, const float* __restrict__ dL_dpix, float* __restrict__ gacc, uint32_t num_tiles,
+    const float* __restrict__ dL_ddepth, const float* __restrict__ dL_dalpha, uint8_t* __restrict__ written,
+    const uint32_t* __restrict__ walk, const uint32_t* __restrict__ walk_count) {
+  render_bwd_body<false, true, true>(ranges, point_list, W, H, rec, bg, final_T, n_contrib, dL_dpix, gacc, num_tiles, dL_ddepth, dL_dalpha, written, walk, walk_count);
+}
+
+}
```

Result: no change. 1125 iters/s (median of 6 runs) (+2.2%).
